# DeepMETv2/DeepMETv2

Measured on AMD Instinct MI355X. Metric: events/sec (4.5k PF cands, k=16), higher is better.
Workload: dtype f32

## Files before the change

### deepmetv2_amd/_lib.py

```python
from __future__ import annotations

import ctypes as C
import os
import threading

_PKG_DIR = os.path.dirname(os.path.abspath(__file__))
LIB_PATH = os.environ.get("DMET_HIP_LIB") or os.path.join(_PKG_DIR, "libdmet_hip.so")

_lock = threading.Lock()
_lib = None

_vp, _i, _i64, _sz, _f, _d = C.c_void_p, C.c_int, C.c_int64, C.c_size_t, C.c_float, C.c_double

SIGNATURES = {
    "dmet_version": (_i, []),
    "dmet_last_error": (C.c_char_p, []),
    "dmet_device_available": (_i, []),
    "dmet_knn_workspace_bytes": (_sz, [_i64, _i, _i, _i]),
    "dmet_knn_f32": (_i, [_vp, _vp, _i, _i64, _i, _i, _vp, _vp, _vp, _sz, _vp]),
    "dmet_knn_local_f32": (_i, [_vp, _vp, _i, _i64, _i, _i, _vp, _vp, _vp, _vp, _sz, _vp]),
    "dmet_knn_periodic_f32": (_i, [_vp, _vp, _i, _i64, _i, _i, _vp, _vp, _vp, _vp, _vp, _sz, _vp]),
    "dmet_knn_xy_workspace_bytes": (_sz, [_i64, _i64, _i, _i, _i]),
    "dmet_knn_xy_f32": (_i, [_vp, _vp, _i64, _vp, _vp, _i64, _i, _i, _i, _vp, _vp, _vp, _vp, _sz, _vp]),
    "dmet_radius_xy_f32": (_i, [_vp, _vp, _i64, _vp, _vp, _i64, _i, _i, _f, _i, _vp, _i, _vp, _vp, _vp]),
    "dmet_edge_features_xy_f32": (_i, [_vp, _vp, _vp, _vp, _i64, _i, _vp, _vp]),
    "dmet_edge_features_xy_bwd_f32": (_i, [_vp, _vp, _vp, _vp, _i64, _i64, _i, _vp, _vp, _vp]),
    "dmet_adamw_f32": (_i, [_vp, _vp, _vp, _vp, _vp, _vp, _i64, _d, _d, _d, _d, _d, _vp]),
    "dmet_adamw_lr_f32": (_i, [_vp, _vp, _vp, _vp, _vp, _vp, _i64, _vp, _d, _d, _d, _d, _vp]),
    "dmet_bn_knn_local_dense_f32": (_i, [_vp, _vp, _vp, _vp, _vp, _vp, _vp, _vp, _i, _i64, _i, _i, _vp, _vp, _vp, _vp, _vp, _i,
                                         _vp, _vp, _vp, _vp, _vp, _sz, _vp]),
    "dmet_knn_local_dense_f32": (_i, [_vp, _vp, _i, _i64, _i, _i, _vp, _vp, _vp, _vp, _vp, _i, _vp, _vp, _vp, _vp, _sz, _vp]),
    "dmet_knn_fallback_stats": (_i, [_vp, _i64, _i, _i, _i, _vp, _vp]),
    "dmet_knn_retry_stats": (_i, [_vp, _i64, _i, _i, _i, _vp, _vp]),
    "dmet_knn_size_hint": (_i, [_i, _i]),
    "dmet_finalize_defer_begin": (_i, []),
    "dmet_finalize_pending": (_i, []),
    "dmet_finalize_flush": (_i, [_vp]),
    "dmet_radius_f32": (_i, [_vp, _vp, _i, _i64, _i, _f, _i, _i, _vp, _vp, _vp]),
    "dmet_radius_counted_f32": (_i, [_vp, _vp, _i, _i64, _i, _f, _i, _i, _vp, _vp, _vp]),
    "dmet_radius_workspace_bytes": (_sz, [_i64]),
    "dmet_radius_windowed_f32": (_i, [_vp, _vp, _i, _i64, _i, _f, _i, _i, _i, _vp, _vp, _vp, _sz, _vp]),
    "dmet_radius_windowed_local_f32": (_i, [_vp, _vp, _i, _i64, _i, _f, _i, _i, _i, _vp, _vp, _vp, _i, _vp, _sz, _vp]),
    "dmet_radius_periodic_f32": (_i, [_vp, _vp, _i, _i64, _i, _f, _i, _i, _i, _vp, _vp, _vp, _vp]),
    "dmet_radius_windowed_periodic_f32": (_i, [_vp, _vp, _i, _i64, _i, _f, _i, _i, _i, _vp, _vp, _vp, _vp, _i, _vp, _sz,
                                               _vp]),
    "dmet_edgeconv_linear_workspace_bytes": (_sz, [_i64, _i]),
    "dmet_edgeconv_linear_max_fwd_f32": (_i, [_vp, _vp, _vp, _i, _i64, _i, _i, _i, _vp, _vp, _vp, _vp, _vp, _sz, _vp]),
    "dmet_edgeconv_fused_lds_f32": (_i, [_vp, _vp, _vp, _i, _i64, _i, _i, _i, _vp, _vp, _vp, _vp, _vp]),
    "dmet_node_linear_split_f32": (_i, [_vp, _i64, _i, _i, _vp, _vp, _vp, _vp, _vp]),
    "dmet_node_linear_split_sliced_f32": (_i, [_vp, _i64, _i, _i, _vp, _vp, _vp, _vp, _vp]),
    "dmet_bn_node_linear_split_f32": (_i, [_vp, _vp, _vp, _vp, _vp, _vp, _vp, _i64, _i, _vp, _vp, _i, _vp, _vp, _vp]),
    "dmet_gather_max_f32": (_i, [_vp, _vp, _vp, _vp, _i, _i64, _i, _i, _vp, _vp, _vp]),
    "dmet_gather_max_counted_f32": (_i, [_vp, _vp, _vp, _vp, _i64, _i, _i, _vp, _vp, _vp]),
    "dmet_gather_max_lds_f32": (_i, [_vp, _vp, _vp, _vp, _i, _i64, _i, _i, _vp, _vp, _vp]),
    "dmet_gather_max_counted_lds_f32": (_i, [_vp, _vp, _vp, _vp, _vp, _i, _i64, _i, _i, _i, _vp, _vp, _vp]),
    "dmet_gather_max_lds_sliced_f32": (_i, [_vp, _vp, _vp, _vp, _vp, _i, _i64, _i, _i, _vp, _vp, _vp]),
    "dmet_gather_max_lds_sliced_cap_f32": (_i, [_vp, _vp, _vp, _vp, _vp, _i, _i64, _i, _i, _vp, _vp, _i64, _vp]),
    "dmet_gather_max_lds16_f32": (_i, [_vp, _vp, _vp, _vp, _vp, _i, _i64, _i, _i, _vp, _vp, _vp]),
    "dmet_edge_mlp2_supported": (_i, [_i, _i, _i, _i]),
    "dmet_edge_mlp2_bf16": (_i, [_vp, _i64, _i, _vp, _i, _vp, _vp, _i, _vp, _vp, _i, _i, _i, _vp, _vp]),
    "dmet_edge_mlp2_bn_workspace_bytes": (_sz, [_i64, _i]),
    "dmet_edge_mlp2_bn_bf16": (_i, [_vp, _i64, _i, _vp, _i, _vp, _vp, _i, _vp, _vp, _i, _i, _i, _vp, _vp, _f, _f, _vp, _vp, _vp,
                                    _i, _vp, _vp, _sz, _vp]),
    "dmet_edge_mlp_f32_supported": (_i, [_i, _i, _i]),
    "dmet_edge_mlp_f32_workspace_bytes": (_sz, [_i64, _i64, _i, _i, _i]),
    "dmet_edge_mlp_fwd_f32": (_i, [_vp, _i64, _i, _vp, _vp, _vp, _i64, _vp, _vp, _i, _vp, _vp, _i, _i, _i, _i, _vp, _vp, _f, _f,
                                   _vp, _vp, _vp, _vp, _vp, _vp, _vp, _vp, _vp, _sz, _vp]),
    "dmet_edge_mlp_bwd_f32": (_i, [_vp, _i64, _i, _vp, _vp, _vp, _i64, _vp, _vp, _vp, _i, _vp, _vp, _i, _i, _i, _i, _vp, _vp,
                                   _vp, _vp, _vp, _vp, _vp, _vp, _vp, _vp, _vp, _vp, _sz, _vp]),
    "dmet_edge_mlp_bf16_supported": (_i, [_i, _i, _i]),
    "dmet_edge_mlp_bf16_workspace_bytes": (_sz, [_i64, _i64, _i, _i, _i]),
    "dmet_edge_mlp_fwd_bf16": (_i, [_vp, _i64, _i, _vp, _vp, _vp, _i64, _vp, _vp, _i, _vp, _vp, _i, _i, _i, _i, _vp, _vp, _f, _f,
                                    _vp, _vp, _vp, _vp, _vp, _vp, _vp, _vp, _vp, _sz, _vp]),
    "dmet_edge_mlp_bwd_bf16": (_i, [_vp, _i64, _i, _vp, _vp, _vp, _i64, _vp, _vp, _vp, _i, _vp, _vp, _i, _i, _i, _i, _vp, _vp,
                                    _vp, _vp, _vp, _vp, _vp, _vp, _vp, _vp, _vp, _vp, _sz, _vp]),
    "dmet_edge_mlp_f16_supported": (_i, [_i, _i, _i]),
    "dmet_edge_mlp_f16_workspace_bytes": (_sz, [_i64, _i64, _i, _i, _i]),
    "dmet_edge_mlp_fwd_f16": (_i, [_vp, _i64, _i, _vp, _vp, _vp, _i64, _vp, _vp, _i, _vp, _vp, _i, _i, _i, _i, _vp, _vp, _f, _f,
                                   _vp, _vp, _vp, _vp, _vp, _vp, _vp, _vp, _vp, _sz, _vp]),
    "dmet_edge_mlp_bwd_f16": (_i, [_vp, _i64, _i, _vp, _vp, _vp, _i64, _vp, _vp, _vp, _i, _vp, _vp, _i, _i, _i, _i, _vp, _vp,
                                   _vp, _vp, _vp, _vp, _vp, _vp, _vp, _vp, _vp, _vp, _sz, _vp]),
    "dmet_table_order_by_count": (_i, [_vp, _vp, _i, _i64, _vp, _vp]),
    "dmet_gather_max_counted_lds_j16_f32": (_i, [_vp, _vp, _vp, _vp, _vp, _vp, _i, _i64, _i, _i, _i, _vp, _vp, _vp]),
    "dmet_gather_max_local_j16_f32": (_i, [_vp, _vp, _vp, _i, _vp, _vp, _vp, _i, _i64, _i, _i, _i, _vp, _vp, _vp]),
    "dmet_gather_max_bwd_j16_f32": (_i, [_vp, _vp, _vp, _i, _i64, _i, _vp, _vp]),
    "dmet_gather_max_mixed_f32": (_i, [_vp, _vp, _vp, _vp, _vp, _i, _i64, _i, _i, _vp, _vp, _vp]),
    "dmet_node_linear_split_bf16": (_i, [_vp, _i64, _i, _i, _vp, _vp, _vp, _vp, _vp]),
    "dmet_gather_max_bf16q": (_i, [_vp, _vp, _vp, _i64, _i, _i, _vp, _vp, _vp]),
    "dmet_gather_max_bwd_f32": (_i, [_vp, _vp, _vp, _vp, _i64, _i, _i, _vp, _vp]),
    "dmet_gather_sum_table_f32": (_i, [_vp, _vp, _vp, _vp, _i64, _i, _i, _i, _vp, _vp, _vp]),
# ... 43 lines not shown
    "dmet_met_loss_f32": (_i, [_vp, _vp, _i, _vp, _vp, _vp]),
    "dmet_met_loss_strided_f32": (_i, [_vp, _vp, _i64, _i, _vp, _vp, _vp]),
    "dmet_met_reduce_bwd_scaled_f32": (_i, [_vp, _vp, _vp, _i64, _vp, _i, _i64, _vp, _vp]),
    "dmet_segment_sum_1d_f32": (_i, [_vp, _vp, _i, _vp, _vp]),
    "dmet_table_degree": (_i, [_vp, _vp, _i64, _i, _vp, _vp]),
    "dmet_table_edges": (_i, [_vp, _vp, _vp, _i64, _i, _i, _vp, _vp, _vp, _vp, _vp]),
    "dmet_batch_to_ptr": (_i, [_vp, _i64, _i, _vp, _vp]),
    "dmet_xty_workspace_bytes": (_sz, [_i64, _i, _i]),
    "dmet_xty_f32": (_i, [_vp, _vp, _i64, _i, _i, _vp, _vp, _sz, _vp]),
    "dmet_onehot_xty_f32": (_i, [_vp, _vp, _i64, _i, _i, _vp, _vp, _sz, _vp]),
    "dmet_gather_max_bwd_lds_f32": (_i, [_vp, _vp, _vp, _vp, _i, _i64, _i, _i, _vp, _vp]),
    "dmet_gather_max_bwd_lds16_f32": (_i, [_vp, _vp, _vp, _vp, _vp, _i, _i64, _i, _i, _vp, _vp]),
    "dmet_gather_max_bwd_lds16_cap_f32": (_i, [_vp, _vp, _vp, _vp, _vp, _i, _i64, _i, _i, _vp, _i64, _vp]),
    "dmet_gather_max_bwd_j16_cap_f32": (_i, [_vp, _vp, _vp, _i, _i64, _i, _vp, _i64, _vp]),
    "dmet_gather_max_bwd_sliced_f32": (_i, [_vp, _vp, _vp, _vp, _vp, _i, _i64, _i, _i, _vp, _i64, _vp]),
    "dmet_gather_max_bwd_j16_sliced_f32": (_i, [_vp, _vp, _vp, _i, _i64, _i, _vp, _i64, _vp]),
    "dmet_edgeconv_linear_bwd_sliced_f32": (_i, [_vp, _vp, _vp, _vp, _i, _vp, _vp, _i64, _i, _vp, _vp, _vp, _vp, _sz, _vp]),
    "dmet_edgeconv_linear_bwd_workspace_bytes": (_sz, [_i64, _i]),
    "dmet_edgeconv_linear_bwd_f32": (_i, [_vp, _vp, _vp, _vp, _vp, _i64, _i, _vp, _vp, _vp, _vp, _sz, _vp]),
    "dmet_edgeconv_linear_bwd_add_f32": (_i, [_vp, _vp, _vp, _vp, _vp, _vp, _i64, _i, _vp, _vp, _vp, _vp, _sz, _vp]),
    "dmet_edgeconv_linear_bwd_add_j16_f32": (_i, [_vp, _vp, _vp, _vp, _vp, _vp, _i64, _i, _vp, _vp, _vp, _vp, _sz, _vp]),
    "dmet_head_fwd_f32": (_i, [_vp, _i64, _vp, _vp, _vp, _vp, _vp, _vp]),
    "dmet_head_bwd_workspace_bytes": (_sz, [_i64]),
    "dmet_head_bwd_f32": (_i, [_vp, _i64] + [_vp] * 10 + [_vp, _sz, _vp]),
    "dmet_bn_workspace_bytes": (_sz, [_i64, _i]),
    "dmet_bn_fwd_f32": (_i, [_vp, _vp, _i64, _i, _vp, _vp, _f, _f, _vp, _vp, _i, _vp, _vp, _vp, _vp, _sz, _vp]),
    "dmet_bn_fwd_tracked_f32": (_i, [_vp, _vp, _i64, _i, _vp, _vp, _f, _f, _vp, _vp, _vp, _i, _vp, _vp, _vp, _vp, _sz, _vp]),
    "dmet_bn_head_fwd_f32": (_i, [_vp, _vp, _vp, _vp, _vp, _vp, _vp, _i64, _vp, _vp, _vp, _vp, _vp, _vp, _vp]),
    "dmet_bn_bwd_stats_f32": (_i, [_vp, _vp, _i64, _i, _vp, _vp, _vp, _vp, _vp, _vp, _vp, _sz, _vp]),
    "dmet_encode_bn_bwd_f32": (_i, [_vp, _i64, _vp, _i64] + [_vp] * 9 + [_vp, _vp] + [_vp] * 5 + [_vp] * 9 + [_vp, _vp, _sz, _vp]),
    "dmet_bn_eval_stats_f32": (_i, [_vp, _vp, _i, _f, _vp, _vp, _vp]),
    "dmet_bn_apply_f32": (_i, [_vp, _vp, _i64, _i, _vp, _vp, _vp, _vp, _vp, _vp]),
    "dmet_bn_stats_f32": (_i, [_vp, _i64, _i, _f, _f, _vp, _vp, _vp, _vp, _vp, _vp, _sz, _vp]),
    "dmet_bn_bwd_f32": (_i, [_vp, _vp, _i64, _i, _vp, _vp, _vp, _vp, _vp, _vp, _vp, _sz, _vp]),
    "dmet_encode_fwd_f32": (_i, [_vp, _i64, _vp, _i64] + [_vp] * 9 + [_vp, _vp]),
    "dmet_encode_bwd_workspace_bytes": (_sz, [_i64]),
    "dmet_encode_bwd_f32": (_i, [_vp, _i64, _vp, _i64] + [_vp] * 9 + [_vp, _vp] + [_vp] * 9 + [_vp, _sz, _vp]),
    "dmet_graclus_workspace_bytes": (_sz, [_i64]),
    "dmet_graclus_f32": (_i, [_vp, _vp, _vp, _vp, _i, _i64, C.c_uint64, _i, _vp, _vp, _vp, _vp, _sz, _vp]),
    "dmet_normalized_cut_workspace_bytes": (_sz, [_i64]),
    "dmet_normalized_cut_f32": (_i, [_vp, _vp, _i64, _i64, _vp, _vp, _vp, _sz, _vp]),
    "dmet_normalized_cut_2d_f32": (_i, [_vp, _vp, _i64, _i64, _vp, _i, _vp, _vp, _sz, _vp]),
    "dmet_pool_pairs_workspace_bytes": (_sz, [_i64, _i]),
    "dmet_pool_pairs_index": (_i, [_vp, _vp, _i, _i64, _vp, _vp, _vp, _sz, _vp]),
    "dmet_pool_pairs_f32": (_i, [_vp, _i64, _i, _vp, _vp, _vp, _i, _i64, _vp, _vp, _vp, _vp, _vp]),
    "dmet_pool_pairs_bwd_f32": (_i, [_vp, _vp, _vp, _vp, _vp, _i64, _i, _i64, _vp, _vp]),
    "dmet_fps_workspace_bytes": (_sz, [_i64, _i, _i]),
    "dmet_fps_f32": (_i, [_vp, _vp, _i, _i64, _i, _vp, _vp, _i64, _vp, _vp, _sz, _vp]),
    "dmet_topk_workspace_bytes": (_sz, [_i64]),
    "dmet_topk_f32": (_i, [_vp, _vp, _i, _i64, _vp, _i64, _vp, _vp, _vp, _sz, _vp]),
    "dmet_select_rows_f32": (_i, [_vp, _vp, _vp, _i64, _i64, _i, _vp, _vp]),
    "dmet_select_rows_bwd_f32": (_i, [_vp, _vp, _vp, _vp, _i64, _i64, _i, _vp, _vp, _vp]),
    "dmet_filter_table": (_i, [_vp, _vp, _vp, _vp, _i64, _i64, _i, _vp, _vp, _vp]),
    "dmet_filter_edges_workspace_bytes": (_sz, [_i64]),
    "dmet_filter_edges_count": (_i, [_vp, _vp, _i64, _vp, _i64, _vp, _vp, _vp, _sz, _vp]),
    "dmet_filter_edges_write": (_i, [_vp, _vp, _i64, _vp, _i64, _vp, _sz, _i64, _vp, _vp, _vp]),
}


class DmetLibraryError(RuntimeError):
    pass


def load() -> C.CDLL:
    global _lib
    if _lib is not None:
# ... 22 lines not shown
```

### deepmetv2_amd/_native.py

```python
from __future__ import annotations

import contextlib
import ctypes
import inspect
import math
import os
from typing import Optional, Tuple

import torch

from . import _lib


def _require_device(*tensors: torch.Tensor) -> torch.device:
    dev = None
    for t in tensors:
        if t is None:
            continue
        if t.device.type != "cuda":
            raise RuntimeError(
                "deepmetv2_amd: operator called with a non-GPU tensor. The HIP extension is the only "
                "implementation (no CPU fallback); move inputs to a ROCm device.")
        if dev is None:
            dev = t.device
# ... 412 lines not shown
    _t = timer.record('node_linear_split', dev)
    with _on(dev):
        _lib.check(L.dmet_bn_node_linear_split_f32(raw.data_ptr(), _ptr(residual), *[v.data_ptr() for v in vec], y.data_ptr(),
                                                   N, 32, W.data_ptr(), _ptr(b), layout, P.data_ptr(), Q.data_ptr(),
                                                   _stream(dev)), "dmet_bn_node_linear_split_f32")
    if _t is not None:
        _t.record(torch.cuda.current_stream(dev))
    return y, P, Q


def _gather_run(dev: torch.device, key: str, note: Optional[str], entry: str, *args) -> None:
    _t = timer.record(key, dev)
    if note is not None:
        _note_gather(note)
    with _on(dev):
        _lib.check(getattr(_lib.load(), entry)(*args, _stream(dev)), entry)
    if _t is not None:
        _t.record(torch.cuda.current_stream(dev))


def _pq_shape(P: torch.Tensor, sliced: bool) -> Tuple[int, int]:
    return (P.shape[1], P.shape[0] * 8) if sliced else (P.shape[0], P.shape[1])


def _check_nbr_local(nbr_local: Optional[torch.Tensor], nbr: torch.Tensor) -> None:
    if nbr_local is not None and (nbr_local.shape != nbr.shape or nbr_local.dtype != torch.int16
                                  or not nbr_local.is_contiguous()):
        raise ValueError("nbr_local must be the contiguous int16 [N, k] table of knn_local()")


def gather_max(P: torch.Tensor, Q: torch.Tensor, nbr: torch.Tensor, ptr: Optional[torch.Tensor],
               want_arg: bool, cnt: Optional[torch.Tensor] = None, lds: bool = False,
               nbr_local: Optional[torch.Tensor] = None, sliced: bool = False, mixed: bool = False,
               max_nodes: Optional[int] = None) -> Tuple[torch.Tensor, Optional[torch.Tensor]]:
    dev = _require_device(P, Q, nbr)
    N, H = _pq_shape(P, sliced)
    k = nbr.shape[1]
    out = torch.empty((N, H), dtype=torch.float32, device=dev)
    arg = torch.empty((N, H), dtype=torch.uint8, device=dev) if want_arg else None
    table = (P.data_ptr(), Q.data_ptr(), nbr.data_ptr())
    local = _ptr(nbr_local)
    events = (ptr.data_ptr(), ptr.numel() - 1) if ptr is not None else (None, 0)
    outs = (out.data_ptr(), arg.data_ptr() if want_arg else None)
    tail = (N, k, H) + outs
    lds_form = ptr is not None and H % 8 == 0 and GATHER_MAX_FORM != "l2-only"
    if mixed and cnt is None and not sliced and ptr is not None and GATHER_MAX_FORM == "auto":
        _check_nbr_local(nbr_local, nbr)
        entry, args = "dmet_gather_max_mixed_f32", table + (local,) + events + tail
        note = ("gather_max_lds_kernel (events <= 5119 nodes: Q slice resident in LDS) + gather_max_mlp_kernel "
                "(larger events: row gathers from L2), chosen per event in one call; row-major P/Q")
    elif sliced and cnt is None:
        if ptr is None or k not in LDS_GATHER_K or GATHER_MAX_FORM == "l2-only":
            raise ValueError("gather_max: slice-major tables are only read by the LDS-resident kernels")
        entry, args = "dmet_gather_max_lds_sliced_cap_f32", table + (local,) + events + tail + (int(max_nodes or 0),)
        note = ("gather_max_lds_kernel (per-event Q slice resident in LDS; slice-major P/Q, "
                + ("uint16 event-local ids)" if nbr_local is not None else "int32 ids)"))
    elif cnt is not None and lds and lds_form:
        entry = "dmet_gather_max_counted_lds_f32"
        args = table + (cnt.data_ptr(),) + events + (N, k, H, 1 if sliced else 0) + outs
        note = ("gather_max_lds_kernel, counted rows (radius table; Q slice resident in LDS"
                + (", slice-major P/Q)" if sliced else ")"))
    elif sliced:
        raise ValueError("gather_max: slice-major tables are only read by the LDS-resident kernels")
    elif cnt is not None:
        entry, args = "dmet_gather_max_counted_f32", table + (cnt.data_ptr(),) + tail
        note = "gather_max_kernel, counted rows (radius table; gathers from L2)"
    elif (lds or GATHER_MAX_FORM == "lds") and lds_form and nbr_local is not None and k in LDS_GATHER_K:
        _check_nbr_local(nbr_local, nbr)
        entry, args = "dmet_gather_max_lds16_f32", table + (local,) + events + tail
        note = "gather_max_lds_kernel (per-event Q slice resident in LDS; row-major P/Q, uint16 ids)"
    elif (lds or GATHER_MAX_FORM == "lds") and lds_form:
        entry, args = "dmet_gather_max_lds_f32", table + events + tail
        note = "gather_max_lds_kernel (per-event Q slice resident in LDS; row-major P/Q, int32 ids)"
    else:
        entry, args = "dmet_gather_max_f32", table + events + tail
        note = "gather_max_mlp_kernel (row gathers from L2; events too large for the LDS image)"
    _gather_run(dev, 'gather_max', note, entry, *args)
    return out, arg


def table_order_by_count(cnt: torch.Tensor, ptr: torch.Tensor) -> torch.Tensor:
    dev = _require_device(cnt, ptr)
    L = _lib.load()
    N = cnt.numel()
    order = torch.empty((N,), dtype=torch.int32, device=dev)
    with _on(dev):
        _lib.check(L.dmet_table_order_by_count(cnt.data_ptr(), ptr.data_ptr(), ptr.numel() - 1, N, order.data_ptr(),
                                               _stream(dev)), "dmet_table_order_by_count")
    return order


def gather_max_counted_j16(P: torch.Tensor, Q: torch.Tensor, nbr: torch.Tensor, cnt: torch.Tensor,
                           order: Optional[torch.Tensor], ptr: torch.Tensor, sliced: bool):
    dev = _require_device(P, Q, nbr, cnt, ptr)
    N, H = _pq_shape(P, sliced)
    k = nbr.shape[1]
    out = torch.empty((N, H), dtype=torch.float32, device=dev)
    argj = torch.empty((N, H), dtype=torch.int16, device=dev)
    _gather_run(dev, 'gather_max', "gather_max_lds_kernel, counted rows (radius table; Q slice resident in LDS, winner ids, "
                "rows ordered by depth" + (", slice-major P/Q)" if sliced else ")"), "dmet_gather_max_counted_lds_j16_f32",
                P.data_ptr(), Q.data_ptr(), nbr.data_ptr(), cnt.data_ptr(), _ptr(order),
                ptr.data_ptr(), ptr.numel() - 1, N, k, H, 1 if sliced else 0, out.data_ptr(), argj.data_ptr())
    return out, argj


def gather_max_local_j16(P: torch.Tensor, Q: torch.Tensor, rows16: torch.Tensor, cnt: torch.Tensor,
                         order: Optional[torch.Tensor], ptr: torch.Tensor, kmax: int, sliced: bool, want_arg: bool = True):
    dev = _require_device(P, Q, rows16, cnt, ptr)
    N, H = _pq_shape(P, sliced)
# ... 1444 lines not shown
                                         ws.numel(), _stream(dev)), "dmet_onehot_xty_f32")
    return C


def _encode_params(params, dev):
    shapes = [(16, 8), (16,), (16, 24), (16,), (32, 32), (32,), (3, 8), (7, 8), (8, 8)]
    if len(params) != 9:
        raise ValueError("encode: expected 9 parameter tensors (Wc, bc, Wk, bk, Wa, ba, Echg, Epdg, Epv)")
    out = []
    for t, shp in zip(params, shapes):
        if tuple(t.shape) != shp:
            raise ValueError(f"encode: parameter of shape {tuple(t.shape)}, expected {shp}")
        if t.device != dev:
            raise ValueError("encode: parameters must be on the device of x")
        out.append(_f32c(t, "param"))
    return out


def _encode_x(x: torch.Tensor, x_cat: torch.Tensor):
    if x.dim() != 2 or x.shape[1] != 8 or x.dtype != torch.float32:
        raise ValueError(f"encode: x_cont must be float32 [N,8], got {tuple(x.shape)} {x.dtype}")
    if x_cat.dim() != 2 or x_cat.shape != (x.shape[0], 3):
        raise ValueError(f"encode: x_cat must be [N,3], got {tuple(x_cat.shape)}")
    if x_cat.dtype == torch.float32:
        if (x.stride(1) == 1 and x_cat.stride(1) == 1 and x_cat.stride(0) == x.stride(0) and x.stride(0) >= 11
                and x_cat.data_ptr() == x.data_ptr() + 32):
            return x, None
        x_cat = x_cat.long()
    if x_cat.dtype != torch.int64:
        raise ValueError(f"encode: x_cat must be int64 (or the float columns 8..10 of x), got {x_cat.dtype}")
    return (x if x.stride(1) == 1 else x.contiguous()), x_cat.contiguous()


def encode_fwd(x_cont: torch.Tensor, x_cat: torch.Tensor, params) -> torch.Tensor:
    dev = _require_device(x_cont, x_cat)
    L = _lib.load()
    x, xc = _encode_x(x_cont, x_cat)
    ps = _encode_params(params, dev)
    N = x.shape[0]
    h = torch.empty((N, 32), dtype=torch.float32, device=dev)
    with _on(dev):
        _lib.check(L.dmet_encode_fwd_f32(x.data_ptr(), x.stride(0), _ptr(xc), N, *[t.data_ptr() for t in ps],
                                         h.data_ptr(), _stream(dev)), "dmet_encode_fwd_f32")
    return h


def encode_bwd(x_cont: torch.Tensor, x_cat: torch.Tensor, params, h: torch.Tensor, g_h: torch.Tensor):
    dev = _require_device(x_cont, x_cat, h, g_h)
    L = _lib.load()
    x, xc = _encode_x(x_cont, x_cat)
    ps = _encode_params(params, dev)
    h = _f32a(h, "h"); g_h = _f32a(g_h, "g_h")
    N = x.shape[0]
    grads = [torch.empty_like(t) for t in ps]
    if N == 0:
        return [g.zero_() for g in grads]
    with _on(dev):
        ws = _ws(L.dmet_encode_bwd_workspace_bytes(N), dev)
        again = _defer_second_use(dev, *params)
        try:
            _lib.check(L.dmet_encode_bwd_f32(x.data_ptr(), x.stride(0), _ptr(xc), N, *[t.data_ptr() for t in ps],
                                             h.data_ptr(), g_h.data_ptr(), *[g.data_ptr() for g in grads], ws.data_ptr(),
                                             ws.numel(), _stream(dev)), "dmet_encode_bwd_f32")
        finally:
            if again:
                _defer_resume()
        _defer_keep(dev, ws, *grads)
    return grads


def encode_bn_bwd(x_cont: torch.Tensor, x_cat: torch.Tensor, params, h: torch.Tensor, g_y: torch.Tensor,
                  gamma: torch.Tensor, mean: torch.Tensor, invstd: torch.Tensor):
    dev = _require_device(x_cont, x_cat, h, g_y)
    L = _lib.load()
    x, xc = _encode_x(x_cont, x_cat)
    ps = _encode_params(params, dev)
    h = _f32c(h, "h"); g_y = _f32c(g_y, "g_y"); gamma = _f32c(gamma.detach(), "gamma")
# ... 34 lines not shown
def bn_fwd(x: torch.Tensor, residual: Optional[torch.Tensor], gamma: torch.Tensor, beta: torch.Tensor, eps: float,
           momentum: float, running_mean: Optional[torch.Tensor], running_var: Optional[torch.Tensor], training: bool,
           num_batches_tracked: Optional[torch.Tensor] = None):
    dev = _require_device(x, gamma, beta)
    L = _lib.load()
    x = _f32a(x, "x")
    N, H = x.shape
    if residual is not None:
        residual = _f32a(residual, "residual")
        if residual.shape != x.shape:
            raise ValueError("bn_fwd: residual must have the shape of x")
    for t in (running_mean, running_var):
        if t is not None and (not t.is_contiguous() or t.dtype != torch.float32 or t.numel() != H):
            raise ValueError("bn_fwd: running statistics must be contiguous float32 [H]")
    gamma = _f32a(gamma, "gamma"); beta = _f32a(beta, "beta")
    y = torch.empty_like(x)
    stats = torch.empty((2, H), dtype=torch.float32, device=dev)
    with _on(dev):
        ws = _ws(L.dmet_bn_workspace_bytes(N, H), dev)
        nbt = None
        if num_batches_tracked is not None and training:
            if num_batches_tracked.dtype != torch.int64 or num_batches_tracked.numel() != 1 or num_batches_tracked.device != dev:
                raise ValueError("bn_fwd: num_batches_tracked must be an int64 scalar on x's device")
            nbt = num_batches_tracked.data_ptr()
        _lib.check(L.dmet_bn_fwd_tracked_f32(x.data_ptr(), _ptr(residual), N, H, gamma.data_ptr(), beta.data_ptr(),
                                             float(eps), float(momentum), _ptr(running_mean), _ptr(running_var), nbt,
                                             1 if training else 0, y.data_ptr(), stats[0].data_ptr(),
                                             stats[1].data_ptr(), ws.data_ptr(), ws.numel(), _stream(dev)),
                   "dmet_bn_fwd_tracked_f32")
    return y, stats[0], stats[1]


def bn_stats(x: torch.Tensor, eps: float, momentum: float, running_mean: Optional[torch.Tensor],
             running_var: Optional[torch.Tensor], num_batches_tracked: Optional[torch.Tensor] = None):
    dev = _require_device(x)
    L = _lib.load()
    x = _f32a(x, "x")
    N, H = x.shape
    stats = torch.empty((2, H), dtype=torch.float32, device=dev)
    with _on(dev):
        ws = _ws(L.dmet_bn_workspace_bytes(N, H), dev)
        _lib.check(L.dmet_bn_stats_f32(x.data_ptr(), N, H, float(eps), float(momentum), _ptr(running_mean),
                                       _ptr(running_var), _ptr(num_batches_tracked),
                                       stats[0].data_ptr(), stats[1].data_ptr(), ws.data_ptr(), ws.numel(), _stream(dev)),
                   "dmet_bn_stats_f32")
    return stats[0], stats[1]


def bn_apply(x: torch.Tensor, residual: Optional[torch.Tensor], gamma: torch.Tensor, beta: torch.Tensor,
             mean: torch.Tensor, invstd: torch.Tensor) -> torch.Tensor:
    dev = _require_device(x, gamma, beta, mean, invstd)
    L = _lib.load()
    x, residual, vec, aligned = _bn_affine_operands("bn_apply", x, residual, gamma, beta, mean, invstd)
    if not aligned:
        x, vec = _aligned16(x), [_aligned16(v) for v in vec]
        residual = _aligned16(residual) if residual is not None else None
    N, H = x.shape
    y = torch.empty_like(x)
    with _on(dev):
        _lib.check(L.dmet_bn_apply_f32(x.data_ptr(), _ptr(residual), N, H, *[v.data_ptr() for v in vec], y.data_ptr(),
                                       _stream(dev)), "dmet_bn_apply_f32")
    return y


def bn_eval_stats(running_mean: torch.Tensor, running_var: torch.Tensor, eps: float):
    dev = _require_device(running_mean, running_var)
    L = _lib.load()
    H = running_mean.numel()
    stats = torch.empty((2, H), dtype=torch.float32, device=dev)
    with _on(dev):
        _lib.check(L.dmet_bn_eval_stats_f32(running_mean.data_ptr(), running_var.data_ptr(), H, float(eps),
                                            stats[0].data_ptr(), stats[1].data_ptr(), _stream(dev)), "dmet_bn_eval_stats_f32")
    return stats[0], stats[1]


def bn_knn_local_dense(raw: torch.Tensor, residual: Optional[torch.Tensor], gamma: torch.Tensor, beta: torch.Tensor,
                       mean: torch.Tensor, invstd: torch.Tensor, ptr: torch.Tensor, k: int, dense=None):
    dev = _require_device(raw, ptr)
# ... 501 lines not shown
```

### deepmetv2_amd/conv.py

```python
from __future__ import annotations

import os
from typing import Callable, Optional, Tuple, Union

import torch

from . import _native
from .cluster import fp16_autocast, knn_table, knn_xy_table
from .graph import BipartiteTable, EdgeList, GraphFuture, NeighborTable, batch_info, edge_list_from_edge_index, lookup_graph
from .scatter import _SegmentMaxRows, _SegmentSumRows
from torch.autograd.function import once_differentiable

_FUSED_WIDTHS = (32, 64)


def _reset(nn_module) -> None:
    if hasattr(nn_module, "reset_parameters"):
        nn_module.reset_parameters()
    elif hasattr(nn_module, "children"):
        for child in nn_module.children():
            _reset(child)


def _as_fusable_linear(nn_module) -> Optional[torch.nn.Linear]:
# ... 55 lines not shown
            if pq is not None and pq[2] is sliced and pq[0].shape[-2 if sliced else 0] == x.shape[0]:
                P, Q = pq[0], pq[1]
            else:
                P, Q = _native.node_linear_split(x, weight, bias, sliced=sliced)
            table.join()
            auto = lds and _native.GATHER_MAX_FORM == "auto"
            ctx.j16 = auto and need_grad and table.nonempty and os.environ.get("DMET_RADIUS_J16", "1") != "0"
            rows16 = table.rows16 is not None and os.environ.get("DMET_RADIUS_IDS", "rows16") == "rows16"
            if ctx.j16 and rows16:
                out, arg = _native.gather_max_local_j16(P, Q, table.rows16, table.cnt, table.order_by_count(), table.ptr,
                                                        table.k, sliced)
            elif ctx.j16:
                out, arg = _native.gather_max_counted_j16(P, Q, table.nbr, table.cnt, table.order_by_count(), table.ptr,
                                                          sliced)
            elif auto and not need_grad and rows16:
                out, arg = _native.gather_max_local_j16(P, Q, table.rows16, table.cnt, table.order_by_count(), table.ptr,
                                                        table.k, sliced, want_arg=False)
            else:
                out, arg = _native.gather_max(P, Q, table.nbr, table.ptr, want_arg=need_grad, cnt=table.cnt, lds=lds,
                                              sliced=sliced)
        elif EDGECONV_FORM == "fused" and _lds_eligible(x, weight, table):
            out, arg = _native.edgeconv_fused_lds(x, weight, bias, table.nbr, table.ptr, want_arg=need_grad)
        else:
            lds = _lds_eligible(x, weight, table)
            mixed = (not lds and _lds_eligible(x, weight, table, any_size=True) and table.max_nodes is not None
                     and os.environ.get("DMET_GATHER_MIXED", "0") == "1")
            sliced = _pq_sliced(lds)
            pq = table.pq
            table.pq = None
            if pq is not None and pq[2] is sliced and pq[0].shape[-2 if sliced else 0] == x.shape[0]:
                P, Q = pq[0], pq[1]
            else:
                P, Q = _native.node_linear_split(x, weight, bias, sliced=sliced)
            out, arg = _native.gather_max(P, Q, table.nbr, table.ptr, want_arg=need_grad, lds=lds,
                                          nbr_local=table.nbr_local, sliced=sliced, mixed=mixed, max_nodes=table.max_nodes)
        if need_grad:
            ctx.save_for_backward(x, weight, arg)
            ctx.table = table
            ctx.has_bias = bias is not None
        if passthrough:
            return out, x.view_as(x)
        return out

    @staticmethod
    def backward(ctx, g_out, g_pass=None):
        _native.no_double_backward("_EdgeConvLinearMax")
        x, weight, arg = ctx.saved_tensors
        table: NeighborTable = ctx.table
        H = x.shape[1]
        g_out = g_out.contiguous()
        fused_node = H == 32 and tuple(weight.shape) == (32, 64) and g_out.dtype == torch.float32
        gqs = fused_node and os.environ.get("DMET_GQ_SLICED", "1") != "0"
        if ctx.j16:
            gQ = _native.gather_max_bwd_j16(g_out, arg, table.ptr, max_nodes=table.max_nodes, sliced=gqs)
        elif H == 32 and g_out.dtype == torch.float32 and table.ptr is not None and GATHER_BWD_FORM != "reverse":
            gQ = _native.gather_max_bwd_lds(g_out, arg, table.nbr, table.ptr, nbr_local=table.nbr_local,
                                            max_nodes=table.max_nodes, sliced=gqs)
        else:
            gqs = False
            rev_ptr, rev_pos = table.reverse()
            gQ = _native.gather_max_bwd(g_out, arg, rev_ptr, rev_pos, table.k)
        if fused_node:
            gx, gW, gb = _native.edgeconv_linear_bwd(x, weight.detach(), g_out,
                                                     None if table.dense else arg, gQ,
                                                     want_bias=ctx.has_bias, g_add=g_pass, gq_sliced=gqs)
            return (gx if ctx.needs_input_grad[0] else None, gW if ctx.needs_input_grad[1] else None,
                    gb if (ctx.has_bias and ctx.needs_input_grad[2]) else None, None, None, None)
        none = 0xFFFF if ctx.j16 else 255
# ... 463 lines not shown
        return f"{self.__class__.__name__}(nn={self.nn})"


class DynamicEdgeConv(EdgeConv):

    def __init__(self, nn: Callable, k: int, aggr: str = "max", num_workers: int = 1, **kwargs):
        super().__init__(nn=nn, aggr=aggr, **kwargs)
        if not isinstance(k, int) or k < 1:
            raise ValueError(f"k must be a positive int, got {k!r}")
        self.k = k
        self.num_workers = num_workers

    def forward(self, x: Union[torch.Tensor, Tuple[torch.Tensor, torch.Tensor]],
                batch: Union[None, torch.Tensor, Tuple[torch.Tensor, torch.Tensor]] = None) -> torch.Tensor:
        if isinstance(x, (tuple, list)):
            if x[1] is not None and x[1] is not x[0]:
                x_src, x_dst = self._check_features(x[0], "x_src"), self._check_features(x[1], "x_dst")
                b_src, b_dst = batch if isinstance(batch, (tuple, list)) else (batch, batch)
                return self._forward_pair(x_src, x_dst, knn_xy_table(x_src, x_dst, self.k, b_src, b_dst))
            x = x[0]
        if isinstance(batch, (tuple, list)):
            batch = batch[0]
        if x.dim() != 2:
            raise ValueError("Static graphs not supported in DynamicEdgeConv")
        if x.dtype == torch.bfloat16 or (x.dtype == torch.float16 and self._takes_fp16()):
            x = x.float()
        if x.dtype != torch.float32:
            raise TypeError(f"x must be float32, got {x.dtype}")
        table = self._take_prebuilt(x)
        if table is None:
            table = knn_table(x, self.k, batch, loop=True, dense=self._dense_request(x))
        return self._forward_table(x, table)

    def forward_with_residual_input(self, x: torch.Tensor, batch: Optional[torch.Tensor] = None):
        if x.dim() != 2 or x.dtype != torch.float32:
            return self.forward(x, batch), x
        table = self._take_prebuilt(x)
        if table is None:
            table = knn_table(x, self.k, batch, loop=True, dense=self._dense_request(x))
        return self._forward_table(x, table, passthrough=True)

    def prebuild_hook(self, batch: Optional[torch.Tensor] = None, graph=None):
        if BN_KNN_FUSE == "0" or self.k > 20 or os.environ.get("DMET_KNN_PATH") == "exact":
            return None

        def build(raw, residual, gamma, beta, mean, invstd):
            if not raw.is_cuda or raw.dim() != 2 or raw.shape[1] != 32 or raw.dtype != torch.float32:
                return None
            info = batch_info(batch, raw.shape[0], raw.device)
            req = self._dense_request(raw)
            dense = (req[0], req[1], req[2](info.max_nodes)) if req is not None else None
            _native.knn_size_hint(info.min_nodes, info.max_nodes)
            out = _native.bn_knn_local_dense(raw, residual, gamma, beta, mean, invstd, info.ptr, self.k, dense)
            if out is None:
                return None
            y, nbr, dist, loc, pq = out
            table = NeighborTable(nbr, info.ptr, dense=False, dist=dist, max_nodes=info.max_nodes, nbr_local=loc)
            table.pq = pq
            self._prebuilt = (y, table)
            return y
        return build

    def _take_prebuilt(self, x: torch.Tensor):
        pre, self._prebuilt = getattr(self, "_prebuilt", None), None
        if pre is not None and pre[0].data_ptr() == x.data_ptr() and pre[0].shape == x.shape:
            return pre[1]
        return None

    def _dense_request(self, x: torch.Tensor):
        if KNN_RIDER == "0" or self.aggr != "max" or EDGECONV_FORM != "split" or x.shape[1] != 32 or not x.is_cuda:
            return None
        lin = _as_fusable_linear(self.nn)
        if lin is None or lin.in_features != 64 or lin.out_features != 32 or self.k not in _native.LDS_GATHER_K:
# ... 13 lines not shown
```

### deepmetv2_amd/csrc/common.h

```cpp
#pragma once
#include <hip/hip_runtime.h>
#include <stdint.h>
#include <stdio.h>
#include <stdlib.h>
#include <string.h>

#include <type_traits>

#include "../../include/dmet.h"

namespace dmet {

constexpr int kWave = 64;
constexpr int kNumXcd = 8;
constexpr float kKnnSentinel = 1e10f;

void set_error(const char *fmt, ...);
int hip_fail(hipError_t e, const char *what);

#define DMET_REQUIRE(cond, ...)                 \
    do {                                        \
        if (!(cond)) {                          \
            ::dmet::set_error(__VA_ARGS__);     \
            return -22;                         \
// ... 23 lines not shown
        const int mid = (lo + hi) >> 1;
        if (ptr[mid] <= i) lo = mid; else hi = mid;
    }
    return lo;
}

__device__ __forceinline__ int xcd_swizzle(int bid, int nblk)
{
    const int q = nblk / kNumXcd, rm = nblk % kNumXcd;
    const int xcd = bid % kNumXcd, idx = bid / kNumXcd;
    const int base = (xcd < rm) ? xcd * (q + 1) : rm * (q + 1) + (xcd - rm) * q;
    return base + idx;
}

constexpr int kEcbPartialFloats = 2 * 1024 + 32;
constexpr int kEncPartialFloats = 3 * 1024 + 64;
constexpr int kHeadPartialFloats = 1024 + 64;
enum { kDeferEdgeConv = 0, kDeferEncoder = 1, kDeferHead = 2 };
struct DeferDesc {
    int kind;
    const float *partial;
    int64_t nparts;
    float *out[9];
};
bool defer_push(const DeferDesc &d);

__device__ __forceinline__ float wave_sum(float v)
{
#pragma unroll
    for (int off = 32; off > 0; off >>= 1) v += __shfl_xor(v, off, 64);
    return v;
}

template <int... Vs, typename F>
bool with_int(int v, F &&f)
{
    return ((v == Vs && (f(std::integral_constant<int, Vs>{}), true)) || ...);
}
template <typename F>
void with_flags(F &&f) { f(); }
template <typename F, typename... Rest>
void with_flags(F &&f, bool b, Rest... rest)
{
    if (b) with_flags([&](auto... c) { f(std::true_type{}, c...); }, rest...);
    else with_flags([&](auto... c) { f(std::false_type{}, c...); }, rest...);
}

}
```

### deepmetv2_amd/csrc/edgeconv.hip

```cpp
#include <stdlib.h>

#include <hip/hip_bf16.h>

#include <type_traits>

#include "common.h"
#include "nls_body.h"

namespace dmet {
namespace {

typedef float f32x16 __attribute__((ext_vector_type(16)));

template <int HIN, int HOUT, bool SLICED = false>
__global__ __launch_bounds__(256) void node_linear_split_kernel(const float *__restrict__ x, int64_t N,
                                                                 const float *__restrict__ W,
                                                                 const float *__restrict__ bias,
                                                                 float *__restrict__ P, float *__restrict__ Q)
{
    __shared__ __attribute__((aligned(16))) float tpose[SLICED ? 4 : 1][SLICED ? kNlsLdsFloats : 1];
    const int wv = __builtin_amdgcn_readfirstlane(threadIdx.x >> 6);
    const int64_t wave = (int64_t)blockIdx.x * (blockDim.x >> 6) + wv;
    const int64_t nwaves = (int64_t)gridDim.x * (blockDim.x >> 6);
    node_linear_split_wave<HIN, HOUT, SLICED>(x, N, W, bias, P, Q, tpose[SLICED ? wv : 0], wave, nwaves, threadIdx.x & 63);
// ... 243 lines not shown
    }
    int4 mine[K4 / 2];
#pragma unroll
    for (int q = 0; q < K4 / 2; ++q) mine[q] = row4[half * (K4 / 2) + q];
#pragma unroll
    for (int q = 0; q < K4 / 2; ++q) {
        int4 other;
        other.x = dpp_swap_pair(mine[q].x); other.y = dpp_swap_pair(mine[q].y);
        other.z = dpp_swap_pair(mine[q].z); other.w = dpp_swap_pair(mine[q].w);
        ids[q] = half ? other : mine[q];
        ids[K4 / 2 + q] = half ? mine[q] : other;
    }
}

template <int K4>
__device__ __forceinline__ void load_ids16_pair(unsigned (&w)[K4], const uint16_t *__restrict__ row, int half)
{
    const unsigned *src = reinterpret_cast<const unsigned *>(row) + half * K4;
    if (K4 % 4 == 0) {
#pragma unroll
        for (int q = 0; q < K4 / 4; ++q) {
            const uint4 v = reinterpret_cast<const uint4 *>(src)[q];
            w[4 * q] = v.x; w[4 * q + 1] = v.y; w[4 * q + 2] = v.z; w[4 * q + 3] = v.w;
        }
    } else if (K4 == 2) {
        const uint2 v = *reinterpret_cast<const uint2 *>(src);
        w[0] = v.x; w[1] = v.y;
    } else {
#pragma unroll
        for (int q = 0; q < K4; ++q) w[q] = src[q];
    }
}

template <bool WITH_ARG, int K4, int GML_MODE, bool IDS16, bool SLICED, int ROWS = kLdsGatherRows, int THREADS = kLdsGatherThreads>
__device__ __forceinline__ void gather_max_lds_segment(
    float4 *__restrict__ qs, const float *__restrict__ P, const float *__restrict__ Q, const int32_t *__restrict__ nbr,
    const uint16_t *__restrict__ nbr16, const int64_t *__restrict__ ptr, int k, int H,
    float *__restrict__ out, uint8_t *__restrict__ arg, int64_t N, int skip_big, const int b, const int sl, const int i0,
    const int i1)
{
    static_assert(K4 >= 1 && K4 <= 8, "k = 4 K4 <= 32");
    constexpr int RPI = THREADS / 2;
    const int lo = (int)ptr[b], hi = (int)ptr[b + 1];
    const int n = hi - lo;
    if (n <= 0 || i0 >= i1) return;
    const int h4 = H / 4;
    const float4 *Q4 = reinterpret_cast<const float4 *>(Q);
    const float4 *P4 = reinterpret_cast<const float4 *>(P);
    const int half = threadIdx.x & 1;
    const int r0 = i0 + (threadIdx.x >> 1);
    const int col4 = sl * 2 + half;
    const float ninf = -__builtin_inff();
    auto pq_at = [&](const int64_t i) -> int64_t { return SLICED ? ((int64_t)sl * N + i) * 2 + half : i * h4 + col4; };

    if (n + 1 > ROWS) {
        if (skip_big) return;
        for (int r = r0; r < i1; r += RPI) {
            const int64_t node = lo + r;
            float4 best = make_float4(ninf, ninf, ninf, ninf);
            int a0 = 255, a1 = 255, a2 = 255, a3 = 255;
            bool any = false;
            for (int s = 0; s < k; ++s) {
                const int j = nbr[node * k + s];
                if (j < 0) continue;
                any = true;
                const float4 v = Q4[pq_at(j)];
                if (v.x > best.x) { best.x = v.x; a0 = s; }
                if (v.y > best.y) { best.y = v.y; a1 = s; }
                if (v.z > best.z) { best.z = v.z; a2 = s; }
                if (v.w > best.w) { best.w = v.w; a3 = s; }
            }
            float4 o = make_float4(0.f, 0.f, 0.f, 0.f);
            if (any) {
                const float4 p = P4[pq_at(node)];
                o = make_float4(p.x + best.x, p.y + best.y, p.z + best.z, p.w + best.w);
            }
            reinterpret_cast<float4 *>(out)[node * h4 + col4] = o;
            if (WITH_ARG)
                reinterpret_cast<uchar4 *>(arg)[node * h4 + col4] =
                    make_uchar4((unsigned char)a0, (unsigned char)a1, (unsigned char)a2, (unsigned char)a3);
        }
        return;
    }

    if (GML_MODE != 1) {
        const int lane = threadIdx.x & 63, wave = threadIdx.x >> 6;
        const int nchunk = (n + 31) / 32;
        for (int c = wave; c < nchunk; c += THREADS / 64) {
            int row = 32 * c + (lane >> 1);
            row = min(row, n - 1);
            const float4 *src = SLICED ? Q4 + ((int64_t)sl * N + lo + row) * 2 + (lane & 1)
                                       : Q4 + (int64_t)(lo + row) * h4 + sl * 2 + (lane & 1);
            __builtin_amdgcn_global_load_lds((const __attribute__((address_space(1))) void *)src,
                                             (__attribute__((address_space(3))) void *)(qs + 64 * c), 16, 0, 0);
        }
    }
    int4 ids[K4];
    unsigned idw[K4];
    float4 pv = make_float4(0.f, 0.f, 0.f, 0.f);
    if (r0 < i1) {
        if constexpr (IDS16) {
            load_ids16_pair<K4>(idw, nbr16 + (int64_t)(lo + r0) * k, half);
        } else {
            const int4 *row4 = reinterpret_cast<const int4 *>(nbr + (int64_t)(lo + r0) * k);
            load_ids_pair<K4>(ids, row4, half);
        }
        pv = P4[pq_at(lo + r0)];
    }
    __builtin_amdgcn_s_waitcnt(0);
    __syncthreads();
    if (threadIdx.x < 2) qs[n * 2 + threadIdx.x] = make_float4(ninf, ninf, ninf, ninf);
    __syncthreads();

    for (int r = r0; r < i1; r += RPI) {
        const int64_t node = lo + r;
        unsigned off[4 * K4];
        if constexpr (IDS16) {
#pragma unroll
            for (int q = 0; q < K4; ++q) {
                const unsigned mine = idw[q], other = (unsigned)dpp_swap_pair((int)mine);
                const unsigned a = half ? other : mine, c = half ? mine : other;
                off[2 * q] = min(a & 0xFFFFu, (unsigned)n) * 2 + half;
                off[2 * q + 1] = min(a >> 16, (unsigned)n) * 2 + half;
                off[2 * K4 + 2 * q] = min(c & 0xFFFFu, (unsigned)n) * 2 + half;
                off[2 * K4 + 2 * q + 1] = min(c >> 16, (unsigned)n) * 2 + half;
            }
        } else {
#pragma unroll
            for (int q = 0; q < K4; ++q) {
                off[4 * q + 0] = min((unsigned)(ids[q].x - lo), (unsigned)n) * 2 + half;
                off[4 * q + 1] = min((unsigned)(ids[q].y - lo), (unsigned)n) * 2 + half;
                off[4 * q + 2] = min((unsigned)(ids[q].z - lo), (unsigned)n) * 2 + half;
                off[4 * q + 3] = min((unsigned)(ids[q].w - lo), (unsigned)n) * 2 + half;
            }
        }
        const float4 p = pv;
        if (r + RPI < i1) {
            if constexpr (IDS16) {
                load_ids16_pair<K4>(idw, nbr16 + (node + RPI) * k, half);
            } else {
                const int4 *row4 = reinterpret_cast<const int4 *>(nbr + (node + RPI) * k);
                load_ids_pair<K4>(ids, row4, half);
            }
            pv = P4[pq_at(node + RPI)];
        }
// ... 42 lines not shown
        for (int q0 = 0; q0 < (GML_MODE == 2 ? 0 : K4); q0 += 2) {
            float4 v[8];
            constexpr int kLastSlot = 4 * K4 - 1;
#pragma unroll
            for (int u = 0; u < 8; ++u) v[u] = qs[off[min(4 * q0 + u, kLastSlot)]];
#pragma unroll
            for (int u = 0; u < 8; ++u) {
                if (4 * q0 + u > kLastSlot) continue;
                if (WITH_ARG) {
                    switch (4 * q0 + u) {
#define DMET_CASE(S_) case S_: DMET_MAX_ARG(bx, a0, v[u].x, S_); DMET_MAX_ARG(by, a1, v[u].y, S_); \
                               DMET_MAX_ARG(bz, a2, v[u].z, S_); DMET_MAX_ARG(bw, a3, v[u].w, S_); break;
                        DMET_CASE(0) DMET_CASE(1) DMET_CASE(2) DMET_CASE(3) DMET_CASE(4) DMET_CASE(5) DMET_CASE(6)
                        DMET_CASE(7) DMET_CASE(8) DMET_CASE(9) DMET_CASE(10) DMET_CASE(11) DMET_CASE(12)
                        DMET_CASE(13) DMET_CASE(14) DMET_CASE(15) DMET_CASE(16) DMET_CASE(17) DMET_CASE(18)
                        DMET_CASE(19) DMET_CASE(20) DMET_CASE(21) DMET_CASE(22) DMET_CASE(23) DMET_CASE(24)
                        DMET_CASE(25) DMET_CASE(26) DMET_CASE(27) DMET_CASE(28) DMET_CASE(29) DMET_CASE(30)
                        DMET_CASE(31)
#undef DMET_CASE
                    }
                } else if ((u & 1) == 0) {
                    asm("v_max3_f32 %0, %0, %1, %2" : "+v"(bx) : "v"(v[u].x), "v"(v[u + 1].x));
                    asm("v_max3_f32 %0, %0, %1, %2" : "+v"(by) : "v"(v[u].y), "v"(v[u + 1].y));
                    asm("v_max3_f32 %0, %0, %1, %2" : "+v"(bz) : "v"(v[u].z), "v"(v[u + 1].z));
                    asm("v_max3_f32 %0, %0, %1, %2" : "+v"(bw) : "v"(v[u].w), "v"(v[u + 1].w));
                }
            }
        }
        }
        const bool any = WITH_ARG ? (a0 != 255) : (bx > ninf);
        float4 o = make_float4(0.f, 0.f, 0.f, 0.f);
        if (any) o = make_float4(p.x + bx, p.y + by, p.z + bz, p.w + bw);
        reinterpret_cast<float4 *>(out)[node * h4 + col4] = o;
        if (WITH_ARG) {
            const uchar4 a = make_uchar4((unsigned char)a0, (unsigned char)a1, (unsigned char)a2, (unsigned char)a3);
            reinterpret_cast<uchar4 *>(arg)[node * h4 + col4] = a;
        }
    }
}

inline int num_cus()
{
    static int cached = 0;
    if (cached == 0) {
        int dev = 0, cus = 0;
        if (hipGetDevice(&dev) == hipSuccess &&
            hipDeviceGetAttribute(&cus, hipDeviceAttributeMultiprocessorCount, dev) == hipSuccess && cus > 0)
            cached = cus;
        else
            cached = 256;
    }
    return cached;
}

template <bool WITH_ARG, int K4, int GML_MODE = 0, bool IDS16 = false, bool SLICED = false, int ROWS = kLdsGatherRows,
          int THREADS = kLdsGatherThreads>
__global__ __launch_bounds__(THREADS) void gather_max_lds_kernel(
    const float *__restrict__ P, const float *__restrict__ Q, const int32_t *__restrict__ nbr,
    const uint16_t *__restrict__ nbr16, const int64_t *__restrict__ ptr, int B, int k, int H,
    float *__restrict__ out, uint8_t *__restrict__ arg, int64_t N, int skip_big, int balanced)
{
    __shared__ __attribute__((aligned(16))) float4 qs[ROWS * 2];
    const int nsl = H / kSliceC;
    if (!balanced) {
        const int grp = blockIdx.x / (kNumXcd * nsl), rem = blockIdx.x % (kNumXcd * nsl);
        const int b = grp * kNumXcd + (rem % kNumXcd);
        const int sl = rem / kNumXcd;
        if (b >= B) return;
        gather_max_lds_segment<WITH_ARG, K4, GML_MODE, IDS16, SLICED, ROWS, THREADS>(qs, P, Q, nbr, nbr16, ptr, k, H, out, arg, N,
                                                                                      skip_big, b, sl, 0, (int)(ptr[b + 1] - ptr[b]));
        return;
    }
    const int64_t L = (int64_t)nsl * N;
    const int c = xcd_swizzle((int)blockIdx.x, (int)gridDim.x);
    int64_t pos = L * c / gridDim.x;
    const int64_t end = L * (c + 1) / gridDim.x;
    while (pos < end) {
        int b0 = 0, b1 = B;
        while (b1 - b0 > 1) {
            const int mid = (b0 + b1) >> 1;
            if ((int64_t)nsl * ptr[mid] <= pos) b0 = mid; else b1 = mid;
        }
        const int64_t lo = ptr[b0];
        const int n = (int)(ptr[b0 + 1] - lo);
        const int64_t rel = pos - (int64_t)nsl * lo;
        const int sl = (int)(rel / n), i0 = (int)(rel - (int64_t)sl * n);
        const int i1 = (int)((end - pos) < (int64_t)(n - i0) ? i0 + (end - pos) : n);
        gather_max_lds_segment<WITH_ARG, K4, GML_MODE, IDS16, SLICED, ROWS, THREADS>(qs, P, Q, nbr, nbr16, ptr, k, H, out, arg, N,
                                                                                      skip_big, b0, sl, i0, i1);
        pos += i1 - i0;
        __syncthreads();
    }
}

template <bool WITH_ARG, bool SLICED, bool ARGJ = false, bool LOC16 = false>
__global__ __launch_bounds__(kLdsGatherThreads) void gather_max_lds_counted_kernel(
    const float *__restrict__ P, const float *__restrict__ Q, const int32_t *__restrict__ nbr,
    const int32_t *__restrict__ cnt, const int64_t *__restrict__ ptr, int B, int kmax, int H,
    float *__restrict__ out, uint8_t *__restrict__ arg, int64_t N, const int32_t *__restrict__ order = nullptr,
    const uint16_t *__restrict__ nbr16 = nullptr, int stride16 = 0)
{
    __shared__ __attribute__((aligned(16))) float4 qs[kLdsGatherRows * 2];
    constexpr int RPI = kLdsGatherThreads / 2;
    const int nsl = H / kSliceC;
    const int grp = blockIdx.x / (kNumXcd * nsl), rem = blockIdx.x % (kNumXcd * nsl);
// ... 553 lines not shown

namespace {

constexpr int kLdsGatherRowsHalf = kLdsGatherRows / 2;
constexpr int kLdsGatherThreadsHalf = kLdsGatherThreads / 2;

enum GatherFamily {
    kGatherL2,
    kGatherLds,
    kGatherCountedLds
};

struct GatherMax {
    const char *entry;
    GatherFamily family;
    const float *P, *Q;
    int64_t N;
    int k, H;
    float *out;
    dmet_stream_t stream;
    const int32_t *nbr = nullptr;
    const uint16_t *nbr16 = nullptr;
    bool rows16 = false;
    int stride16 = 0;
    const int32_t *cnt = nullptr;
    const int32_t *order = nullptr;
    const int64_t *ptr = nullptr;
    int B = 0;
    void *arg = nullptr;
    bool arg16 = false;
    bool pq_sliced = false;
    int skip_big = 0;
    int64_t max_nodes = 0;
};

int gather_max_launch(const GatherMax &r)
{
    const int64_t N = r.N;
    const int k = r.k, H = r.H, B = r.B;
    const bool k_mlp = k == 8 || k == 16 || k == 32, k_lds = k_mlp || k == 20;
    const GatherFamily fam = (r.skip_big && !(H == 32 && k_mlp && B != 0)) ? kGatherL2 : r.family;
    DMET_REQUIRE(N >= 0 && N < (int64_t)2147483647, "%s: N out of range", r.entry);
    DMET_REQUIRE(k >= 1 && k <= 255, "%s: k=%d not in [1,255] (arg is uint8, 255 = none)", r.entry, k);
    DMET_REQUIRE(!r.rows16 || (r.stride16 >= k && r.stride16 % 8 == 0), "%s: kmax=%d stride16=%d", r.entry, k, r.stride16);
    DMET_REQUIRE(r.max_nodes >= 0, "%s: max_nodes=%lld", r.entry, (long long)r.max_nodes);
    DMET_REQUIRE(fam == kGatherL2 || (H >= kSliceC && H % kSliceC == 0 && H <= DMET_MAX_H), "%s: H=%d must be a multiple of %d",
                 r.entry, H, kSliceC);
    if (N == 0 || (fam != kGatherL2 && B == 0)) return 0;
    const void *table = r.rows16 ? static_cast<const void *>(r.nbr16) : r.nbr;
    DMET_REQUIRE(r.P && r.Q && table && r.out && (fam == kGatherL2 || r.ptr) && (fam != kGatherCountedLds || r.cnt) &&
                     (r.arg || !r.arg16 || r.rows16),
                 "%s: null pointer", r.entry);
    DMET_REQUIRE(aligned16(r.P) && aligned16(r.Q) && aligned16(r.out) && (fam != kGatherLds || aligned16(r.nbr)) &&
                     (fam == kGatherL2 || aligned16(r.nbr16)) && (!r.arg16 || (reinterpret_cast<uintptr_t>(r.arg) & 7u) == 0),
                 "%s: pointers must be 16-B (uint16 winners: 8-B) aligned", r.entry);
    hipStream_t st = as_stream(r.stream);
    uint8_t *arg = static_cast<uint8_t *>(r.arg);
    const int nsl = H / kSliceC;
    const int64_t per_event = (int64_t)((B + kNumXcd - 1) / kNumXcd) * kNumXcd * nsl;

    auto launch_mlp = [&](bool only_big) {
        with_int<8, 16, 32>(k, [&](auto kk) {
            constexpr int K4 = decltype(kk)::value / 4;
            with_flags([&](auto with_arg, auto big) {
                hipLaunchKernelGGL((gather_max_mlp_kernel<32, with_arg(), K4, big()>), dim3((unsigned)((N + 31) / 32)), dim3(256),
                                   0, st, r.P, r.Q, r.nbr, N, r.out, arg, r.ptr, B, kLdsGatherRows);
            }, arg != nullptr, only_big);
        });
    };

    if (fam == kGatherCountedLds) {
        with_flags([&](auto with_arg, auto sliced, auto ids, auto loc16) {
            if constexpr (ids() ? (with_arg() || loc16()) : !loc16())
                hipLaunchKernelGGL((gather_max_lds_counted_kernel<with_arg(), sliced(), ids(), loc16()>),
                                   dim3((unsigned)per_event), dim3(kLdsGatherThreads), 0, st, r.P, r.Q, r.nbr, r.cnt, r.ptr, B, k, H,
                                   r.out, arg, N, r.order, r.nbr16, r.stride16);
        }, arg != nullptr, r.pq_sliced, r.arg16, r.rows16);
        DMET_LAUNCH_CHECK(!r.arg16 ? "gather_max_lds_counted_kernel" : !r.rows16 ? "gather_max_lds_counted_kernel (winner ids)"
                          : arg     ? "gather_max_lds_counted_kernel (uint16 rows)"
                                    : "gather_max_lds_counted_kernel (uint16 rows, no winners)");
        return 0;
    }
    if (fam == kGatherLds && k_lds) {
        const bool half = r.pq_sliced && r.nbr16 && r.max_nodes > 0 && r.max_nodes + 1 <= kLdsGatherRowsHalf &&
                          !env_is("DMET_GATHER_HALF_IMAGE", "0");
        const int cus = num_cus();
        const int64_t units = (int64_t)B * nsl;
        int balanced = units * 16 <= (int64_t)cus * 9 || (units > cus && units % cus != 0 && units % cus <= cus / 8);
        if (const char *e = getenv("DMET_GATHER_BALANCED")) balanced = atoi(e) != 0;
        if (half) balanced = 0;
        int64_t blocks = per_event;
        if (balanced) {
            blocks = cus;
            const int64_t most = ((int64_t)nsl * N + 63) / 64;
            if (blocks > most) blocks = most;
        }
        bool timed = false;
#ifdef DMET_KNN_EXPERIMENT
        const char *e = (!half && arg && r.nbr16 && k == 16) ? getenv("DMET_GML_MODE") : nullptr;
        timed = with_int<1, 2>(e ? atoi(e) : 0, [&](auto mode) {
            hipLaunchKernelGGL((gather_max_lds_kernel<true, 4, decltype(mode)::value, true>), dim3((unsigned)blocks),
                               dim3(kLdsGatherThreads), 0, st, r.P, r.Q, r.nbr, r.nbr16, r.ptr, B, k, H, r.out, arg, N, r.skip_big,
                               balanced);
        });
#endif
        if (!timed)
            with_int<8, 16, 20, 32>(k, [&](auto kk) {
                constexpr int K4 = decltype(kk)::value / 4;
                with_flags([&](auto with_arg, auto ids16, auto sliced, auto small) {
                    constexpr int ROWS = small() ? kLdsGatherRowsHalf : kLdsGatherRows;
                    constexpr int THREADS = small() ? kLdsGatherThreadsHalf : kLdsGatherThreads;
                    if constexpr (!small() || (ids16() && sliced()))
                        hipLaunchKernelGGL((gather_max_lds_kernel<with_arg(), K4, 0, ids16(), sliced(), ROWS, THREADS>),
                                           dim3((unsigned)blocks), dim3(THREADS), 0, st, r.P, r.Q, r.nbr, r.nbr16, r.ptr, B, k, H, r.out,
                                           arg, N, r.skip_big, balanced);
                }, arg != nullptr, r.nbr16 != nullptr, r.pq_sliced, half);
            });
        DMET_LAUNCH_CHECK(half ? "gather_max_lds_kernel (80 KB image)" : "gather_max_lds_kernel");
        if (!r.skip_big) return 0;
        launch_mlp(true);
        DMET_LAUNCH_CHECK("gather_max_mlp_kernel (large events)");
        return 0;
    }
    DMET_REQUIRE(!r.pq_sliced, "%s: k=%d (slice-major tables need k in {8,16,20,32})", r.entry, k);
    bool built = true;
    if (H == 32 && !r.cnt && k_mlp && aligned16(r.nbr))
        launch_mlp(false);
    else
        built = with_int<16, 32, 64, 128>(H, [&](auto hh) {
            constexpr int HH = decltype(hh)::value, NPB = 256 / (HH / 4);
            with_flags([&](auto with_arg) {
                hipLaunchKernelGGL((gather_max_kernel<HH, with_arg()>), dim3((unsigned)((N + NPB - 1) / NPB)), dim3(256), 0, st, r.P,
                                   r.Q, r.nbr, r.cnt, N, k, r.out, arg);
            }, arg != nullptr);
        });
    DMET_REQUIRE(built, "%s: unsupported H=%d (16/32/64/128)", r.entry, H);
    DMET_LAUNCH_CHECK("gather_max_kernel");
    return 0;
}

}

extern "C" int dmet_gather_max_f32(const float *P, const float *Q, const int32_t *nbr, const int64_t *ptr, int B,
                                   int64_t N, int k, int H, float *out, uint8_t *arg, dmet_stream_t stream)
{
    (void)ptr; (void)B;
    GatherMax r{"dmet_gather_max_f32", kGatherL2, P, Q, N, k, H, out, stream};
    r.nbr = nbr; r.arg = arg;
    return gather_max_launch(r);
// ... 18 lines not shown
extern "C" int dmet_gather_max_lds16_f32(const float *P, const float *Q, const int32_t *nbr, const uint16_t *nbr_local,
                                         const int64_t *ptr, int B, int64_t N, int k, int H, float *out,
                                         uint8_t *arg, dmet_stream_t stream)
{
    GatherMax r{"dmet_gather_max_lds16_f32", kGatherLds, P, Q, N, k, H, out, stream};
    r.nbr = nbr; r.nbr16 = nbr_local; r.ptr = ptr; r.B = B; r.arg = arg;
    return gather_max_launch(r);
}

extern "C" int dmet_gather_max_mixed_f32(const float *P, const float *Q, const int32_t *nbr, const uint16_t *nbr_local,
                                         const int64_t *ptr, int B, int64_t N, int k, int H, float *out,
                                         uint8_t *arg, dmet_stream_t stream)
{
    GatherMax r{"dmet_gather_max_mixed_f32", kGatherLds, P, Q, N, k, H, out, stream};
    r.nbr = nbr; r.nbr16 = nbr_local; r.ptr = ptr; r.B = B; r.arg = arg; r.skip_big = 1;
    return gather_max_launch(r);
}

extern "C" int dmet_gather_max_lds_sliced_f32(const float *P, const float *Q, const int32_t *nbr,
                                              const uint16_t *nbr_local, const int64_t *ptr, int B, int64_t N, int k,
                                              int H, float *out, uint8_t *arg, dmet_stream_t stream)
{
    GatherMax r{"dmet_gather_max_lds_sliced_f32", kGatherLds, P, Q, N, k, H, out, stream};
    r.nbr = nbr; r.nbr16 = nbr_local; r.ptr = ptr; r.B = B; r.arg = arg; r.pq_sliced = true;
    return gather_max_launch(r);
}

extern "C" int dmet_gather_max_lds_sliced_cap_f32(const float *P, const float *Q, const int32_t *nbr,
                                                  const uint16_t *nbr_local, const int64_t *ptr, int B, int64_t N, int k,
                                                  int H, float *out, uint8_t *arg, int64_t max_nodes, dmet_stream_t stream)
{
    GatherMax r{"dmet_gather_max_lds_sliced_cap_f32", kGatherLds, P, Q, N, k, H, out, stream};
    r.nbr = nbr; r.nbr16 = nbr_local; r.ptr = ptr; r.B = B; r.arg = arg; r.pq_sliced = true; r.max_nodes = max_nodes;
    return gather_max_launch(r);
}

extern "C" int dmet_gather_max_counted_lds_f32(const float *P, const float *Q, const int32_t *nbr, const int32_t *cnt,
                                               const int64_t *ptr, int B, int64_t N, int k, int H, int pq_sliced,
                                               float *out, uint8_t *arg, dmet_stream_t stream)
{
    GatherMax r{"dmet_gather_max_counted_lds_f32", kGatherCountedLds, P, Q, N, k, H, out, stream};
    r.nbr = nbr; r.cnt = cnt; r.ptr = ptr; r.B = B; r.arg = arg; r.pq_sliced = pq_sliced != 0;
    return gather_max_launch(r);
}

extern "C" int dmet_gather_max_counted_lds_j16_f32(const float *P, const float *Q, const int32_t *nbr, const int32_t *cnt,
                                                   const int32_t *order, const int64_t *ptr, int B, int64_t N, int k,
                                                   int H, int pq_sliced, float *out, uint16_t *argj,
                                                   dmet_stream_t stream)
{
    GatherMax r{"dmet_gather_max_counted_lds_j16_f32", kGatherCountedLds, P, Q, N, k, H, out, stream};
    r.nbr = nbr; r.cnt = cnt; r.order = order; r.ptr = ptr; r.B = B; r.arg = argj; r.arg16 = true; r.pq_sliced = pq_sliced != 0;
    return gather_max_launch(r);
}

extern "C" int dmet_gather_max_local_j16_f32(const float *P, const float *Q, const uint16_t *nbr16, int stride16,
                                             const int32_t *cnt, const int32_t *order, const int64_t *ptr, int B,
                                             int64_t N, int kmax, int H, int pq_sliced, float *out, uint16_t *argj,
                                             dmet_stream_t stream)
{
    GatherMax r{"dmet_gather_max_local_j16_f32", kGatherCountedLds, P, Q, N, kmax, H, out, stream};
    r.nbr16 = nbr16; r.rows16 = true; r.stride16 = stride16; r.cnt = cnt; r.order = order; r.ptr = ptr; r.B = B;
    r.arg = argj; r.arg16 = true; r.pq_sliced = pq_sliced != 0;
    return gather_max_launch(r);
}

// ... 261 lines not shown
```

### deepmetv2_amd/csrc/encoder.hip

```cpp
#include <stdlib.h>

#include "bn_affine.h"
#include "common.h"

namespace dmet {
namespace {

typedef float f32x16 __attribute__((ext_vector_type(16)));

#define ENC_PARAMS                                                                                                  \
    const float *__restrict__ Wc, const float *__restrict__ bc, const float *__restrict__ Wk,                      \
        const float *__restrict__ bk, const float *__restrict__ Wa, const float *__restrict__ ba,                  \
        const float *__restrict__ Echg, const float *__restrict__ Epdg, const float *__restrict__ Epv
#define ENC_ARGS Wc, bc, Wk, bk, Wa, ba, Echg, Epdg, Epv

__device__ __forceinline__ float elu(float z) { return z > 0.0f ? z : (__expf(z) - 1.0f); }

__device__ __forceinline__ void cat_indices(const int64_t *__restrict__ xcat, const float *__restrict__ row, int64_t i,
                                            int &ichg, int &ipdg, int &ipv)
{
    long long c = xcat ? xcat[i * 3 + 0] : (long long)row[8];
    const long long chg = xcat ? xcat[i * 3 + 1] : (long long)row[9];
    const long long pv = xcat ? xcat[i * 3 + 2] : (long long)row[10];
    c = c < 0 ? -c : c;
// ... 27 lines not shown
        z2[o] = b;
    }
#pragma unroll
    for (int o = 0; o < 16; ++o) { joint[o] = elu(z2[o]); joint[16 + o] = elu(z1[o]); }
#pragma unroll
    for (int o = 0; o < 32; ++o) {
        float a = ba[o];
#pragma unroll
        for (int f = 0; f < 32; ++f) a = __builtin_fmaf(Wa[o * 32 + f], joint[f], a);
        z3[o] = a;
    }
}

__global__ __launch_bounds__(256, 2) void encode_fwd_kernel(const float *__restrict__ x, int64_t x_stride,
                                                          const int64_t *__restrict__ xcat, int64_t N,
                                                          ENC_PARAMS, float *__restrict__ h)
{
    const int64_t i = (int64_t)blockIdx.x * blockDim.x + threadIdx.x;
    if (i >= N) return;
    const float *row = x + i * x_stride;
    float xc[8];
#pragma unroll
    for (int f = 0; f < 8; ++f) xc[f] = row[f];
    int ichg, ipdg, ipv;
    cat_indices(xcat, row, i, ichg, ipdg, ipv);
    float cat24[24], z1[16], z2[16], joint[32], z3[32];
    encode_node(ENC_ARGS, xc, ichg, ipdg, ipv, cat24, z1, z2, joint, z3);
    float4 *o = reinterpret_cast<float4 *>(h + i * 32);
#pragma unroll
    for (int c = 0; c < 8; ++c)
        o[c] = make_float4(elu(z3[4 * c]), elu(z3[4 * c + 1]), elu(z3[4 * c + 2]), elu(z3[4 * c + 3]));
}

__global__ __launch_bounds__(256) void encode_fwd_mfma_kernel(const float *__restrict__ x, int64_t x_stride,
                                                               const int64_t *__restrict__ xcat, int64_t N, ENC_PARAMS,
                                                               float *__restrict__ h)
{
    const int lane = threadIdx.x & 63, r = lane & 31, hh = lane >> 5;
    const int64_t wave = (int64_t)blockIdx.x * (blockDim.x >> 6) + __builtin_amdgcn_readfirstlane((int)(threadIdx.x >> 6));
    const int64_t nwaves = (int64_t)gridDim.x * (blockDim.x >> 6);
    const int64_t ntiles = (N + 31) / 32;
    float w12[16], w3[16], b12[16], b3[16];
#pragma unroll
    for (int s = 0; s < 16; ++s) {
        const int f = (s & 3) + 8 * (s >> 2) + 4 * hh;
        const float *src = r < 16 ? Wk + r * 24 + min(f, 23) : Wc + (r - 16) * 8 + max(f - 24, 0);
        const bool keep = r < 16 ? f < 24 : f >= 24;
        const float a = *src;
        w12[s] = keep ? a : 0.0f;
        w3[s] = Wa[r * 32 + f];
        const float *bsrc = f < 16 ? bk + f : bc + (f - 16);
        b12[s] = *bsrc;
        b3[s] = ba[f];
    }
    struct Raw { float c[4]; long long k0, k1, k2; };
    auto load_raw = [&](const int64_t tile, Raw &q) __attribute__((always_inline)) {
        const int64_t node = tile * 32 + r;
        const int64_t i = node < N ? node : N - 1;
        const float *row = x + i * x_stride;
#pragma unroll
        for (int u = 0; u < 4; ++u) q.c[u] = row[4 * hh + u];
        if (xcat) { q.k0 = xcat[i * 3 + 0]; q.k1 = xcat[i * 3 + 1]; q.k2 = xcat[i * 3 + 2]; }
        else { q.k0 = (long long)row[8]; q.k1 = (long long)row[9]; q.k2 = (long long)row[10]; }
    };
    auto load_tables = [&](const Raw &q, float (&in)[16]) __attribute__((always_inline)) {
        long long c = q.k0 < 0 ? -q.k0 : q.k0;
        const long long table[7] = {1, 2, 11, 13, 22, 130, 211};
#pragma unroll
        for (int t = 0; t < 7; ++t) c = (c == table[t]) ? (long long)t : c;
        const int ipdg = (int)min(max(c, 0ll), 6ll), ichg = (int)min(max(q.k1 + 1, 0ll), 2ll), ipv = (int)min(max(q.k2, 0ll), 7ll);
        const float4 e0 = *reinterpret_cast<const float4 *>(Echg + ichg * 8 + 4 * hh);
        const float4 e1 = *reinterpret_cast<const float4 *>(Epdg + ipdg * 8 + 4 * hh);
        const float4 e2 = *reinterpret_cast<const float4 *>(Epv + ipv * 8 + 4 * hh);
        in[0] = e0.x; in[1] = e0.y; in[2] = e0.z; in[3] = e0.w; in[4] = e1.x; in[5] = e1.y; in[6] = e1.z; in[7] = e1.w;
        in[8] = e2.x; in[9] = e2.y; in[10] = e2.z; in[11] = e2.w;
#pragma unroll
        for (int u = 0; u < 4; ++u) in[12 + u] = q.c[u];
    };
    Raw raw;
    float in[16], nxt[16];
    if (wave < ntiles) { load_raw(wave, raw); load_tables(raw, in); }
    if (wave + nwaves < ntiles) load_raw(wave + nwaves, raw);
    for (int64_t tile = wave; tile < ntiles; tile += nwaves) {
        const int64_t node = tile * 32 + r;
        if (tile + nwaves < ntiles) load_tables(raw, nxt);
        if (tile + 2 * nwaves < ntiles) load_raw(tile + 2 * nwaves, raw);
        f32x16 acc;
#pragma unroll
        for (int e = 0; e < 16; ++e) acc[e] = b12[e];
#pragma unroll
        for (int s = 0; s < 16; ++s) acc = __builtin_amdgcn_mfma_f32_32x32x2f32(w12[s], in[s], acc, 0, 0, 0);
        float joint[16];
#pragma unroll
        for (int e = 0; e < 16; ++e) joint[e] = elu(acc[e]);
#pragma unroll
        for (int e = 0; e < 16; ++e) acc[e] = b3[e];
#pragma unroll
        for (int s = 0; s < 16; ++s) acc = __builtin_amdgcn_mfma_f32_32x32x2f32(w3[s], joint[s], acc, 0, 0, 0);
        if (node < N) {
            float4 *o = reinterpret_cast<float4 *>(h + node * 32 + 4 * hh);
#pragma unroll
            for (int g = 0; g < 4; ++g)
                o[2 * g] = make_float4(elu(acc[4 * g]), elu(acc[4 * g + 1]), elu(acc[4 * g + 2]), elu(acc[4 * g + 3]));
        }
#pragma unroll
        for (int u = 0; u < 16; ++u) in[u] = nxt[u];
    }
}

constexpr int kEncTiles = 3;
constexpr int kEncBwdWaves = 4;
constexpr int kEncPartial = kEncTiles * 1024 + 64;

__device__ __forceinline__ void enc_wave_sync()
{
    __builtin_amdgcn_fence(__ATOMIC_RELEASE, "wavefront");
    __builtin_amdgcn_wave_barrier();
    __builtin_amdgcn_fence(__ATOMIC_ACQUIRE, "wavefront");
}

__device__ __forceinline__ void tile_mma(f32x16 &acc, const float *__restrict__ A, const float *__restrict__ Bm, int lane)
{
    const int c = lane & 31, hh = lane >> 5;
#pragma unroll 8
    for (int s = 0; s < 32; ++s) {
        const int node = 2 * s + hh;
        acc = __builtin_amdgcn_mfma_f32_32x32x2f32(A[node * 33 + c], Bm[node * 33 + c], acc, 0, 0, 0);
    }
}

__device__ __forceinline__ void tile_mma_onehot(f32x16 &acc, const int *__restrict__ packed, const float *__restrict__ Bm,
                                                int lane)
{
    const int c = lane & 31, hh = lane >> 5;
    int sh, mask, tgt;
    if (c < 3) { sh = 0; mask = 3; tgt = c; }
    else if (c < 10) { sh = 2; mask = 7; tgt = c - 3; }
    else if (c < 18) { sh = 5; mask = 7; tgt = c - 10; }
    else { sh = 0; mask = 0; tgt = 1; }
#pragma unroll 8
// ... 389 lines not shown
    s = 0.0f;
#pragma unroll
    for (int q = 0; q < 32; ++q) s += red[q][e];
    const int t = idx / 1024, r = (idx % 1024) / 32, c = idx % 32;
    if (t == 0) g.Wa[r * 32 + c] = s;
    else if (t == 1) {
        if (r < 16 && c < 24) g.Wk[r * 24 + c] = s;
        else if (r >= 16 && c >= 24) g.Wc[(r - 16) * 8 + (c - 24)] = s;
    } else if (t == 2) {
        if (r < 3 && c < 8) g.Echg[r * 8 + c] = s;
        else if (r >= 3 && r < 10 && c >= 8 && c < 16) g.Epdg[(r - 3) * 8 + (c - 8)] = s;
        else if (r >= 10 && r < 18 && c >= 16 && c < 24) g.Epv[(r - 10) * 8 + (c - 16)] = s;
    } else if (r == 0) g.ba[c] = s;
    else if (c < 16) g.bk[c] = s;
    else g.bc[c - 16] = s;
}

inline int64_t enc_nodes_per_wave(int64_t N, int64_t *nwaves)
{
    const int64_t target_waves = 2048;
    int64_t npw = (N + target_waves - 1) / target_waves;
#ifdef DMET_ENC_NPW_UP
    npw = (npw + 63) / 64 * 64;
#else
    npw = npw / 64 * 64;
#endif
    if (npw < 64) npw = 64;
    int64_t nw = (N + npw - 1) / npw;
    nw = (nw + kEncBwdWaves - 1) / kEncBwdWaves * kEncBwdWaves;
    *nwaves = nw;
    return npw;
}

thread_local EncBnBwd g_enc_bnb{nullptr, nullptr, nullptr, nullptr, nullptr};
thread_local bool g_enc_bnb_done = false;

}
}

using namespace dmet;

extern "C" int dmet_encode_fwd_f32(const float *x, int64_t x_stride, const int64_t *xcat, int64_t N, const float *Wc, const float *bc,
                                   const float *Wk, const float *bk, const float *Wa, const float *ba,
                                   const float *Echg, const float *Epdg, const float *Epv, float *h,
                                   dmet_stream_t stream)
{
    DMET_REQUIRE(N >= 0 && x_stride >= 8, "dmet_encode_fwd_f32: bad sizes");
    if (N == 0) return 0;
    DMET_REQUIRE(x && Wc && bc && Wk && bk && Wa && ba && Echg && Epdg && Epv && h, "dmet_encode_fwd_f32: null pointer");
    DMET_REQUIRE(xcat || x_stride >= 11, "dmet_encode_fwd_f32: x_cat == NULL needs rows of at least 11 columns (x_stride=%lld)", (long long)x_stride);
    DMET_REQUIRE(aligned16(h), "dmet_encode_fwd_f32: h must be 16-B aligned");
    const int64_t blocks = (N + 255) / 256;
    DMET_REQUIRE(blocks < (1ll << 31), "dmet_encode_fwd_f32: too many nodes");
    const int form = env_is("DMET_ENCODER_FWD", "valu") ? 0 : 1;
    if (form == 1 && aligned16(Echg) && aligned16(Epdg) && aligned16(Epv)) {
        const int64_t tiles = (N + 31) / 32;
        int64_t grid = (tiles + 3) / 4;
        int gmax = 512;
        if (const char *e = getenv("DMET_ENC_GRID")) { gmax = atoi(e); if (gmax < 1) gmax = 512; }
        if (grid > gmax) grid = gmax;
        hipLaunchKernelGGL(encode_fwd_mfma_kernel, dim3((unsigned)grid), dim3(256), 0, as_stream(stream), x, x_stride, xcat, N,
                           ENC_ARGS, h);
        DMET_LAUNCH_CHECK("encode_fwd_mfma_kernel");
        return 0;
    }
    hipLaunchKernelGGL(encode_fwd_kernel, dim3((unsigned)blocks), dim3(256), 0, as_stream(stream), x, x_stride, xcat, N, ENC_ARGS, h);
    DMET_LAUNCH_CHECK("encode_fwd_kernel");
    return 0;
}

extern "C" size_t dmet_encode_bwd_workspace_bytes(int64_t N)
{
    if (N <= 0) return 0;
    int64_t nw;
    (void)enc_nodes_per_wave(N, &nw);
    return sizeof(float) * (size_t)nw * kEncPartial + 512;
}

extern "C" int dmet_encode_bwd_f32(const float *x, int64_t x_stride, const int64_t *xcat, int64_t N, const float *Wc, const float *bc,
                                   const float *Wk, const float *bk, const float *Wa, const float *ba,
                                   const float *Echg, const float *Epdg, const float *Epv, const float *h,
                                   const float *g_h, float *gWc, float *gbc, float *gWk, float *gbk, float *gWa,
                                   float *gba, float *gEchg, float *gEpdg, float *gEpv, void *ws, size_t ws_bytes,
                                   dmet_stream_t stream)
{
    DMET_REQUIRE(N > 0 && x_stride >= 8, "dmet_encode_bwd_f32: bad sizes");
    DMET_REQUIRE((xcat || x_stride >= 11) && x && Wc && bc && Wk && bk && Wa && ba && Echg && Epdg && Epv && h && g_h && gWc && gbc && gWk && gbk &&
                     gWa && gba && gEchg && gEpdg && gEpv && ws,
                 "dmet_encode_bwd_f32: null pointer");
    DMET_REQUIRE(ws_bytes >= dmet_encode_bwd_workspace_bytes(N), "dmet_encode_bwd_f32: workspace too small");
    DMET_REQUIRE(aligned16(h) && aligned16(g_h), "dmet_encode_bwd_f32: h / g_h must be 16-B aligned");
    int64_t nw;
    const int64_t npw = enc_nodes_per_wave(N, &nw);
    float *partial = reinterpret_cast<float *>((reinterpret_cast<uintptr_t>(ws) + 255u) & ~(uintptr_t)255u);
    hipStream_t st = as_stream(stream);
    const int form = env_is("DMET_ENCODER_BWD", "valu") ? 0 : 1;
    int64_t nparts = nw / kEncBwdWaves;
    if (form == 1 && aligned16(Echg) && aligned16(Epdg) && aligned16(Epv) && aligned16(g_h) && aligned16(h)) {
        const int64_t tiles = (N + 31) / 32;
        int64_t grid = (tiles + kEncBwdWaves - 1) / kEncBwdWaves;
// ... 54 lines not shown
```

### deepmetv2_amd/csrc/norm.hip

```cpp
#include "bn_affine.h"
#include "common.h"

namespace dmet {
namespace {

constexpr int kBnBlocks = 512;
constexpr int kBnThreads = 256;

template <int MODE>
__global__ __launch_bounds__(kBnThreads) void bn_reduce_kernel(const float *__restrict__ x, const float *__restrict__ g,
                                                               int64_t N, int H, const float *__restrict__ stat_a,
                                                               const float *__restrict__ stat_b, int64_t rows_per_block,
                                                               float *__restrict__ partial)
{
    __shared__ float4 red0[kBnThreads], red1[kBnThreads];
    const int h4 = H / 4;
    const int rpb = kBnThreads / h4;
    const int tid = threadIdx.x;
    const int c4 = tid % h4, rr = tid / h4;
    const int64_t lo = (int64_t)blockIdx.x * rows_per_block, hi = min(N, lo + rows_per_block);
    float4 a = make_float4(0.f, 0.f, 0.f, 0.f), b = a;
    float4 sa = a, sb = make_float4(1.f, 1.f, 1.f, 1.f);
    if (rr < rpb) {
        if (MODE == 0) sa = reinterpret_cast<const float4 *>(x)[c4];
// ... 44 lines not shown
    __syncthreads();
    s0 = 0.0; s1 = 0.0;
    if (grp == 0)
        for (int q = 0; q < 16; ++q) { s0 += g0[q][c]; s1 += g1[q][c]; }
}

__global__ __launch_bounds__(1024) void bn_fwd_finalize_kernel(const float *__restrict__ partial, int nblocks,
                                                             const float *__restrict__ x, int64_t N, int H, float eps,
                                                             float momentum, float *__restrict__ running_mean,
                                                             float *__restrict__ running_var,
                                                             float *__restrict__ save_mean,
                                                             float *__restrict__ save_invstd,
                                                             int64_t *__restrict__ num_batches_tracked)
{
    double s0, s1;
    bn_combine(partial, nblocks, H, s0, s1);
    const int c = threadIdx.x;
    if (c == 0 && num_batches_tracked) *num_batches_tracked += 1;
    if (c >= H) return;
    const double shift = (double)x[c];
    const double m = s0 / (double)N;
    double var = s1 / (double)N - m * m;
    if (var < 0.0) var = 0.0;
    const double mean = shift + m;
    save_mean[c] = (float)mean;
    save_invstd[c] = (float)(1.0 / sqrt(var + (double)eps));
    if (running_mean) {
        const double unbiased = N > 1 ? var * (double)N / (double)(N - 1) : var;
        running_mean[c] = (float)((1.0 - (double)momentum) * (double)running_mean[c] + (double)momentum * mean);
        running_var[c] = (float)((1.0 - (double)momentum) * (double)running_var[c] + (double)momentum * unbiased);
    }
}

__global__ __launch_bounds__(64) void bn_eval_stats_kernel(const float *__restrict__ running_mean,
                                                           const float *__restrict__ running_var, int H, float eps,
                                                           float *__restrict__ save_mean,
                                                           float *__restrict__ save_invstd)
{
    const int c = threadIdx.x;
    if (c >= H) return;
    save_mean[c] = running_mean[c];
    save_invstd[c] = (float)(1.0 / sqrt((double)running_var[c] + (double)eps));
}

__global__ __launch_bounds__(256) void bn_apply_kernel(const float *__restrict__ x, const float *__restrict__ res,
                                                       int64_t N, int H, const float *__restrict__ gamma,
                                                       const float *__restrict__ beta, const float *__restrict__ mean,
                                                       const float *__restrict__ invstd, float *__restrict__ y)
{
    const BnAffine a{x, res, gamma, beta, mean, invstd};
    const int h4 = H / 4;
    const int64_t total = N * h4;
    for (int64_t t = (int64_t)blockIdx.x * blockDim.x + threadIdx.x; t < total; t += (int64_t)gridDim.x * blockDim.x) {
        const float4 v = reinterpret_cast<const float4 *>(x)[t];
        const BnAffine4 c = bn_affine_load4(a, (int)(t % h4));
        float4 o = bn_affine4(v, c.mu, c.scale, c.beta);
        if (res) o = bn_add4(o, reinterpret_cast<const float4 *>(res)[t]);
        reinterpret_cast<float4 *>(y)[t] = o;
    }
}

__global__ __launch_bounds__(1024) void bn_bwd_finalize_kernel(const float *__restrict__ partial, int nblocks, int64_t N,
                                                             int H, float *__restrict__ g_gamma,
                                                             float *__restrict__ g_beta, float *__restrict__ mean_g,
                                                             float *__restrict__ mean_gx)
{
// ... 72 lines not shown
                           (const float *)nullptr, (const float *)nullptr, rpb, partial);
        DMET_LAUNCH_CHECK("bn_reduce_kernel<0>");
        hipLaunchKernelGGL(bn_fwd_finalize_kernel, dim3(1), dim3(1024), 0, st, partial, nb, x, N, H, eps, momentum,
                           running_mean, running_var, save_mean, save_invstd, num_batches_tracked);
        DMET_LAUNCH_CHECK("bn_fwd_finalize_kernel");
    } else {
        hipLaunchKernelGGL(bn_eval_stats_kernel, dim3(1), dim3(64), 0, st, (const float *)running_mean,
                           (const float *)running_var, H, eps, save_mean, save_invstd);
        DMET_LAUNCH_CHECK("bn_eval_stats_kernel");
    }
    return dmet_bn_apply_f32(x, residual, N, H, gamma, beta, save_mean, save_invstd, y, stream);
}

extern "C" int dmet_bn_stats_f32(const float *x, int64_t N, int H, float eps, float momentum, float *running_mean,
                                 float *running_var, int64_t *num_batches_tracked, float *save_mean, float *save_invstd,
                                 void *ws, size_t ws_bytes, dmet_stream_t stream)
{
    DMET_REQUIRE(bn_shape_ok(H), "dmet_bn_stats_f32: H=%d must be a multiple of 4 in [4,64]", H);
    DMET_REQUIRE(N > 0, "dmet_bn_stats_f32: N=%lld", (long long)N);
    DMET_REQUIRE(x && save_mean && save_invstd && ws, "dmet_bn_stats_f32: null pointer");
    DMET_REQUIRE(aligned16(x) && aligned16(save_mean) && aligned16(save_invstd), "dmet_bn_stats_f32: pointers must be 16-byte aligned");
    DMET_REQUIRE(ws_bytes >= dmet_bn_workspace_bytes(N, H), "dmet_bn_stats_f32: workspace too small");
    DMET_REQUIRE((running_mean == nullptr) == (running_var == nullptr), "dmet_bn_stats_f32: running_mean/var go together");
    hipStream_t st = as_stream(stream);
    float *partial = reinterpret_cast<float *>((reinterpret_cast<uintptr_t>(ws) + 255u) & ~(uintptr_t)255u);
    int64_t rpb;
    const int nb = bn_blocks(N, &rpb);
    hipLaunchKernelGGL((bn_reduce_kernel<0>), dim3(nb), dim3(kBnThreads), 0, st, x, (const float *)nullptr, N, H,
                       (const float *)nullptr, (const float *)nullptr, rpb, partial);
    DMET_LAUNCH_CHECK("bn_reduce_kernel<0>");
    hipLaunchKernelGGL(bn_fwd_finalize_kernel, dim3(1), dim3(1024), 0, st, partial, nb, x, N, H, eps, momentum, running_mean,
                       running_var, save_mean, save_invstd, num_batches_tracked);
    DMET_LAUNCH_CHECK("bn_fwd_finalize_kernel");
    return 0;
}

extern "C" int dmet_bn_fwd_f32(const float *x, const float *residual, int64_t N, int H, const float *gamma,
                               const float *beta, float eps, float momentum, float *running_mean, float *running_var,
                               int training, float *y, float *save_mean, float *save_invstd, void *ws, size_t ws_bytes,
                               dmet_stream_t stream)
{
    return dmet_bn_fwd_tracked_f32(x, residual, N, H, gamma, beta, eps, momentum, running_mean, running_var, nullptr,
                                   training, y, save_mean, save_invstd, ws, ws_bytes, stream);
}

extern "C" int dmet_bn_bwd_f32(const float *x, const float *g_y, int64_t N, int H, const float *gamma,
                               const float *save_mean, const float *save_invstd, float *g_x, float *g_gamma,
                               float *g_beta, void *ws, size_t ws_bytes, dmet_stream_t stream)
{
    DMET_REQUIRE(bn_shape_ok(H), "dmet_bn_bwd_f32: H=%d must be a multiple of 4 in [4,64]", H);
    DMET_REQUIRE(N > 0, "dmet_bn_bwd_f32: N=%lld", (long long)N);
    DMET_REQUIRE(x && g_y && gamma && save_mean && save_invstd && g_x && g_gamma && g_beta && ws,
                 "dmet_bn_bwd_f32: null pointer");
    DMET_REQUIRE(aligned16(x) && aligned16(g_y) && aligned16(g_x) && aligned16(gamma) && aligned16(save_mean) &&
                     aligned16(save_invstd),
                 "dmet_bn_bwd_f32: pointers must be 16-byte aligned");
    DMET_REQUIRE(ws_bytes >= dmet_bn_workspace_bytes(N, H), "dmet_bn_bwd_f32: workspace too small");
    hipStream_t st = as_stream(stream);
    float *partial = reinterpret_cast<float *>((reinterpret_cast<uintptr_t>(ws) + 255u) & ~(uintptr_t)255u);
    float *mean_g = partial + (size_t)kBnBlocks * 2 * H, *mean_gx = mean_g + H;
    int64_t rpb;
    const int nb = bn_blocks(N, &rpb);
    hipLaunchKernelGGL((bn_reduce_kernel<1>), dim3(nb), dim3(kBnThreads), 0, st, x, g_y, N, H, save_mean, save_invstd,
                       rpb, partial);
    DMET_LAUNCH_CHECK("bn_reduce_kernel<1>");
    hipLaunchKernelGGL(bn_bwd_finalize_kernel, dim3(1), dim3(1024), 0, st, partial, nb, N, H, g_gamma, g_beta, mean_g,
// ... 65 lines not shown
```

### deepmetv2_amd/dense.py

```python
from __future__ import annotations

from typing import Optional

import os

import torch

from . import _native


class _Linear(torch.autograd.Function):
    @staticmethod
    def forward(ctx, x, weight, bias):
        ctx.save_for_backward(x, weight)
        ctx.has_bias = bias is not None
        return torch.addmm(bias, x, weight.t()) if bias is not None else x @ weight.t()

    @staticmethod
    def backward(ctx, g):
        _native.no_double_backward("_Linear")
        x, weight = ctx.saved_tensors
        g = g.contiguous()
        gx = g @ weight if ctx.needs_input_grad[0] else None
        gw = _native.xty(g, x) if ctx.needs_input_grad[1] else None
        gb = g.sum(0) if (ctx.has_bias and ctx.needs_input_grad[2]) else None
        return gx, gw, gb


class _Embedding(torch.autograd.Function):
    @staticmethod
    def forward(ctx, index, weight):
        ctx.save_for_backward(index)
        ctx.rows = weight.shape[0]
        return weight.index_select(0, index)

    @staticmethod
    def backward(ctx, g):
        _native.no_double_backward("_Embedding")
        (index,) = ctx.saved_tensors
        return None, _native.onehot_xty(index, g.contiguous(), ctx.rows)


def linear(x: torch.Tensor, weight: torch.Tensor, bias: Optional[torch.Tensor] = None) -> torch.Tensor:
    if x.dim() != 2 or weight.shape[0] > 64 or weight.shape[1] > 64 or x.dtype != torch.float32:
        return torch.nn.functional.linear(x, weight, bias)
    return _Linear.apply(x, weight, bias)


def embedding(index: torch.Tensor, weight: torch.Tensor) -> torch.Tensor:
    if weight.shape[0] > 64 or weight.shape[1] > 64 or index.dim() != 1:
        return torch.nn.functional.embedding(index, weight)
    return _Embedding.apply(index, weight)


class _Encode(torch.autograd.Function):

    @staticmethod
    def forward(ctx, x_cont, x_cat, *params):
        h = _native.encode_fwd(x_cont, x_cat, [p.detach() for p in params])
        ctx.save_for_backward(x_cont, x_cat, h, *params)
        return h

    @staticmethod
    def backward(ctx, g_h):
        _native.no_double_backward("_Encode")
        x_cont, x_cat, h, *params = ctx.saved_tensors
        grads = _native.encode_bwd(x_cont, x_cat, [p.detach() for p in params], h, g_h.contiguous())
        return (None, None, *grads)


def encode(x_cont: torch.Tensor, x_cat: torch.Tensor, *params: torch.Tensor) -> torch.Tensor:
    return _Encode.apply(x_cont, x_cat, *params)


def _bn_forward(x, residual, gamma, beta, running_mean, running_var, training, momentum, eps, tracked, next_build):
    if next_build is None:
        return _native.bn_fwd(x, residual, gamma, beta, eps, momentum, running_mean, running_var, training,
                              num_batches_tracked=tracked)
    if training:
        mean, invstd = _native.bn_stats(x, eps, momentum, running_mean, running_var, tracked)
    else:
        mean, invstd = _native.bn_eval_stats(running_mean, running_var, eps)
    y = next_build(x, residual, gamma, beta, mean, invstd)
    if y is None:
        y = _native.bn_apply(x, residual, gamma, beta, mean, invstd)
    return y, mean, invstd


class _BatchNorm(torch.autograd.Function):

    @staticmethod
    def forward(ctx, x, residual, weight, bias, running_mean, running_var, training, momentum, eps, tracked=None,
                next_build=None):
        fused = next_build is not None and x.is_cuda and x.shape[1] == 32 and (training or running_mean is not None)
        y, mean, invstd = _bn_forward(x, residual, weight.detach(), bias.detach(), running_mean, running_var, training,
                                      momentum, eps, tracked, next_build if fused else None)
        ctx.save_for_backward(x, weight, mean, invstd)
        ctx.training = training
        ctx.has_residual = residual is not None
        return y

    @staticmethod
    def backward(ctx, g_y):
        _native.no_double_backward("_BatchNorm")
        x, weight, mean, invstd = ctx.saved_tensors
        g_y = g_y.contiguous()
        if ctx.training:
            g_x, g_w, g_b = _native.bn_bwd(x, g_y, weight.detach(), mean, invstd)
        else:
            scale = weight.detach() * invstd
            g_x = g_y * scale
            g_w = (g_y * (x - mean) * invstd).sum(0)
            g_b = g_y.sum(0)
        return g_x, (g_y if ctx.has_residual else None), g_w, g_b, None, None, None, None, None, None, None


ENC_BN_FUSE = os.environ.get("DMET_ENC_BN_FUSE", "1")


class _EncodeBN(torch.autograd.Function):

    @staticmethod
    def forward(ctx, x_cont, x_cat, weight, bias, running_mean, running_var, momentum, eps, tracked, next_build, *params):
        h = _native.encode_fwd(x_cont, x_cat, [p.detach() for p in params])
        y, mean, invstd = _bn_forward(h, None, weight.detach(), bias.detach(), running_mean, running_var, True, momentum, eps,
                                      tracked, next_build)
        ctx.save_for_backward(x_cont, x_cat, h, weight, mean, invstd, *params)
        return y

    @staticmethod
    def backward(ctx, g_y):
        _native.no_double_backward("_EncodeBN")
        x_cont, x_cat, h, weight, mean, invstd, *params = ctx.saved_tensors
        g_y = g_y.contiguous()
        ps = [p.detach() for p in params]
        res = _native.encode_bn_bwd(x_cont, x_cat, ps, h, g_y, weight.detach(), mean, invstd)
        if res is None:
            g_h, g_w, g_b = _native.bn_bwd(h, g_y, weight.detach(), mean, invstd)
            grads = _native.encode_bwd(x_cont, x_cat, ps, h, g_h)
        else:
            grads, g_w, g_b = res
        return (None, None, g_w, g_b, None, None, None, None, None, None, *grads)


def encode_bn(x_cont: torch.Tensor, x_cat: torch.Tensor, bn: torch.nn.BatchNorm1d, next_build, *params: torch.Tensor):
    ok = (ENC_BN_FUSE != "0" and x_cont.is_cuda and bn.training and bn.affine and bn.momentum is not None
          and bn.track_running_stats and bn.num_features == 32 and x_cont.shape[0] > 1)
    if not ok:
        return batch_norm(encode(x_cont, x_cat, *params), bn, next_build=next_build)
    return _EncodeBN.apply(x_cont, x_cat, bn.weight, bn.bias, bn.running_mean, bn.running_var, float(bn.momentum),
                           float(bn.eps), bn.num_batches_tracked, next_build, *params)


def batch_norm(x: torch.Tensor, bn: torch.nn.BatchNorm1d, residual: Optional[torch.Tensor] = None,
               next_build=None) -> torch.Tensor:
    H = x.shape[1] if x.dim() == 2 else -1
    ok = (x.dim() == 2 and x.dtype == torch.float32 and H % 4 == 0 and 4 <= H <= 64 and bn.affine
          and bn.momentum is not None and x.shape[0] > 1 and (bn.training or bn.track_running_stats))
    if not ok:
        own = getattr(bn, "_torch_forward", None)
        y = own(x) if own is not None else bn(x)
        return y if residual is None else residual + y
    training = bn.training or not bn.track_running_stats
    rm = bn.running_mean if bn.track_running_stats else None
    rv = bn.running_var if bn.track_running_stats else None
    tracked = bn.num_batches_tracked if (bn.training and bn.track_running_stats) else None
    return _BatchNorm.apply(x, residual, bn.weight, bn.bias, rm, rv, training, float(bn.momentum), float(bn.eps), tracked,
                            next_build)


_HEAD_PREBUILT = [None]
HEAD_FUSE = os.environ.get("DMET_BN_HEAD_FUSE", "1")


def head_prebuild_hook(W1: torch.Tensor, b1: torch.Tensor, W2: torch.Tensor, b2: torch.Tensor):
    if HEAD_FUSE == "0":
        return None

    def build(raw, residual, gamma, beta, mean, invstd):
        if not raw.is_cuda or raw.dim() != 2 or raw.shape[1] != 32 or raw.dtype != torch.float32:
            return None
        res = _native.bn_head_fwd(raw, residual, gamma, beta, mean, invstd,
                                  [W1.detach(), b1.detach(), W2.detach(), b2.detach()])
        if res is None:
            return None
        _HEAD_PREBUILT[0] = res
        return res[0]
    return build


class _Head(torch.autograd.Function):

    @staticmethod
    def forward(ctx, emb, W1, b1, W2, b2):
        pre, _HEAD_PREBUILT[0] = _HEAD_PREBUILT[0], None
        if pre is not None and pre[0].data_ptr() == emb.data_ptr() and pre[0].shape == emb.shape:
            out = pre[1]
        else:
            out = _native.head_fwd(emb, [W1.detach(), b1.detach(), W2.detach(), b2.detach()])
# ... 15 lines not shown
```

### deepmetv2_amd/graph.py

```python
from __future__ import annotations

import weakref
from typing import Dict, Optional, Tuple

import torch

from . import _native


class BatchInfo:
    __slots__ = ("ptr", "num_events", "num_nodes", "max_nodes", "min_nodes", "inferred")

    def __init__(self, ptr: torch.Tensor, num_events: int, num_nodes: int, max_nodes: Optional[int] = None,
                 min_nodes: Optional[int] = None, inferred: bool = False):
        self.ptr = ptr
        self.num_events = num_events
        self.num_nodes = num_nodes
        self.max_nodes = max_nodes
        self.min_nodes = min_nodes
        self.inferred = inferred


_batch_registry: Dict[int, Tuple[weakref.ref, int, BatchInfo]] = {}

# ... 178 lines not shown
    src = src64.to(torch.int32).contiguous()
    rowptr, perm = _reverse_of_column(tgt, num_nodes)
    ident = torch.arange(E, dtype=torch.int32, device=dev)
    if num_src is None:
        grouped, lo, hi = torch.stack([(perm[:E] == ident).all().to(torch.int64), edge_index.min(),
                                       edge_index.max()]).tolist()
        if lo < 0 or hi >= num_nodes:
            raise ValueError(f"edge_index node ids must lie in [0, {num_nodes}), found {lo if lo < 0 else hi}")
    else:
        grouped, lo, hi, slo, shi = torch.stack([(perm[:E] == ident).all().to(torch.int64), tgt64.min(), tgt64.max(),
                                                 src64.min(), src64.max()]).tolist()
        if lo < 0 or hi >= num_nodes:
            raise ValueError(f"edge_index target ids must lie in [0, {num_nodes}), found {lo if lo < 0 else hi}")
        if slo < 0 or shi >= num_src:
            raise ValueError(f"edge_index source ids must lie in [0, {num_src}), found {slo if slo < 0 else shi}")
    if grouped:
        return EdgeList(src, tgt, rowptr, num_nodes, None, num_src=num_src)
    p = perm[:E].to(torch.int64)
    return EdgeList(src[p].contiguous(), tgt[p].contiguous(), rowptr, num_nodes, perm[:E], num_src=num_src)


class NeighborTable:

    def __init__(self, nbr: Optional[torch.Tensor], ptr: Optional[torch.Tensor], dense: bool, dist: Optional[torch.Tensor] = None,
                 max_nodes: Optional[int] = None, cnt: Optional[torch.Tensor] = None,
                 nbr_local: Optional[torch.Tensor] = None, nonempty: bool = False,
                 rows16: Optional[torch.Tensor] = None, full_rows: bool = False, shape: Optional[Tuple[int, int]] = None):
        if nbr is None and (shape is None or rows16 is None or cnt is None or ptr is None):
            raise ValueError("NeighborTable without an int32 table needs shape, rows16, cnt and ptr")
        self._nbr = nbr
        self.full_rows = full_rows
        self._pending = None
        self.pq = None
        self.rows16 = rows16
        self.nonempty = nonempty
        self._order = None
        self.nbr_local = nbr_local
        self.ptr = ptr
        self.max_nodes = max_nodes
        self.cnt = cnt
        self.num_nodes, self.k = (nbr.shape if nbr is not None else shape)
        self.dense = dense
        self.dist = dist
        self._rev = None
        self._rp = None
        self._rp_full = None
        self._edges = None
        self._edge_index = {}

    @property
    def nbr(self) -> torch.Tensor:
        if self._nbr is None:
            self.join()
            N, k = self.num_nodes, self.k
            counts = (self.ptr[1:] - self.ptr[:-1])
            lo = torch.repeat_interleave(self.ptr[:-1], counts, output_size=N).to(torch.int32).view(-1, 1)
            loc = self.rows16[:, :k].to(torch.int32) & 0xFFFF
            slot = torch.arange(k, device=loc.device, dtype=torch.int32).view(1, -1)
            self._nbr = torch.where(slot < self.cnt.view(-1, 1), loc + lo, torch.full_like(loc, -1)).contiguous()
        return self._nbr

    def has_int32_table(self) -> bool:
        return self._nbr is not None

    def join(self) -> "NeighborTable":
        if self._pending is not None:
# ... 162 lines not shown
```

### deepmetv2_amd/model.py

```python
from __future__ import annotations

import os
from typing import Optional

import torch
from torch import nn

from . import dense
from .conv import DynamicEdgeConv, EdgeConv
from .scatter import met_loss, met_loss_from_weights, met_reduce

PDG_CLASSES = (1, 2, 11, 13, 22, 130, 211)


def _run(seq: nn.Sequential, x: torch.Tensor) -> torch.Tensor:
    for layer in seq:
        x = dense.linear(x, layer.weight, layer.bias) if isinstance(layer, nn.Linear) else layer(x)
    return x


class GraphMETNetwork(nn.Module):
    def __init__(self, continuous_dim: int, cat_dim: int, output_dim: int = 1, hidden_dim: int = 32,
                 conv_depth: int = 1, graph: str = "static", k: int = 16, edge_dtype=None):
        super().__init__()
        if graph not in ("static", "dynamic"):
            raise ValueError("graph must be 'static' or 'dynamic'")
        q, h = hidden_dim // 4, hidden_dim // 2
        self.graph, self.k = graph, k
        self.fused_encoder = os.environ.get("DMET_FUSED_ENCODER", "1") != "0"
        self.embed_charge = nn.Embedding(3, q)
        self.embed_pdgid = nn.Embedding(len(PDG_CLASSES), q)
        self.embed_pv = nn.Embedding(8, q)
        self.embed_continuous = nn.Sequential(nn.Linear(continuous_dim, h), nn.ELU())
        self.embed_categorical = nn.Sequential(nn.Linear(3 * q, h), nn.ELU())
        self.encode_all = nn.Sequential(nn.Linear(hidden_dim, hidden_dim), nn.ELU())
        self.bn_all = nn.BatchNorm1d(hidden_dim)
        self.conv_continuous = nn.ModuleList()
        for _ in range(conv_depth):
            message = nn.Sequential(nn.Linear(2 * hidden_dim, hidden_dim))
            conv = DynamicEdgeConv(nn=message, k=k) if graph == "dynamic" else EdgeConv(nn=message).jittable()
            conv.compute_dtype = edge_dtype
            self.conv_continuous.append(nn.ModuleList([conv, nn.BatchNorm1d(hidden_dim)]))
        self.output = nn.Sequential(nn.Linear(hidden_dim, h), nn.ELU(), nn.Linear(h, output_dim))
        self.pdgs = list(PDG_CLASSES)

    def _fused_encoder_ok(self, x_cont: torch.Tensor, x_cat: torch.Tensor) -> bool:
        return (self.fused_encoder and x_cont.dtype == torch.float32 and x_cont.shape[1] == 8
                and x_cat.shape[1] == 3 and self.encode_all[0].weight.shape == (32, 32)
                and list(self.pdgs) == list(PDG_CLASSES) and not x_cont.requires_grad)

    def _next_build(self, layer: int, batch, graph=None):
        if layer >= len(self.conv_continuous):
            return None
        hook = getattr(self.conv_continuous[layer][0], "prebuild_hook", None)
        if hook is None:
            return None
        return hook(batch) if self.graph == "dynamic" else hook(batch, graph=graph)

    def embed(self, x_cont: torch.Tensor, x_cat: torch.Tensor, batch=None, fuse_next: bool = False, graph=None) -> torch.Tensor:
        if self._fused_encoder_ok(x_cont, x_cat):
            lc, lk, la = self.embed_continuous[0], self.embed_categorical[0], self.encode_all[0]
            return dense.encode_bn(x_cont, x_cat, self.bn_all, self._next_build(0, batch, graph) if fuse_next else None,
                                   lc.weight, lc.bias, lk.weight, lk.bias, la.weight, la.bias,
                                   self.embed_charge.weight, self.embed_pdgid.weight, self.embed_pv.weight)
        if x_cat.is_floating_point():
            x_cat = x_cat.long()
        e_cont = _run(self.embed_continuous, x_cont)
        e_chrg = dense.embedding(x_cat[:, 1] + 1, self.embed_charge.weight)
        e_pv = dense.embedding(x_cat[:, 2], self.embed_pv.weight)
        pdg = x_cat[:, 0].abs()
        for cls, val in enumerate(self.pdgs):
            pdg = torch.where(pdg == val, torch.full_like(pdg, cls), pdg)
        e_pdg = dense.embedding(pdg, self.embed_pdgid.weight)
        e_cat = _run(self.embed_categorical, torch.cat([e_chrg, e_pdg, e_pv], dim=1))
        return dense.batch_norm(_run(self.encode_all, torch.cat([e_cat, e_cont], dim=1)), self.bn_all)

    def _fused_head_ok(self, emb: torch.Tensor) -> bool:
        l1, l2 = self.output[0], self.output[2]
        return (self.fused_encoder and emb.dtype == torch.float32 and emb.shape[1] == 32 and l1.bias is not None
                and l2.bias is not None and tuple(l1.weight.shape) == (16, 32) and tuple(l2.weight.shape) == (1, 16))

    def forward(self, x_cont, x_cat, edge_index, batch, apply_sigmoid: bool = False):
        emb = self.embed(x_cont, x_cat, batch, fuse_next=True, graph=edge_index)
        for layer, (conv, norm) in enumerate(self.conv_continuous):
            msg, res = conv.forward_with_residual_input(emb, batch if self.graph == "dynamic" else edge_index)
            nb = self._next_build(layer + 1, batch, edge_index)
            if nb is None and layer + 1 == len(self.conv_continuous) and apply_sigmoid and self._fused_head_ok(res):
                l1, l2 = self.output[0], self.output[2]
                nb = dense.head_prebuild_hook(l1.weight, l1.bias, l2.weight, l2.bias)
            emb = dense.batch_norm(msg, norm, residual=res, next_build=nb)
        if apply_sigmoid and self._fused_head_ok(emb):
            l1, l2 = self.output[0], self.output[2]
            return dense.head(emb, l1.weight, l1.bias, l2.weight, l2.bias)
        out = _run(self.output, emb).squeeze(-1)
        return torch.sigmoid(out) if apply_sigmoid else out


class Net(nn.Module):

    def __init__(self, continuous_dim: int, categorical_dim: int, graph: str = "static", k: int = 16, edge_dtype=None):
        super().__init__()
        self.graphnet = GraphMETNetwork(continuous_dim, categorical_dim, output_dim=1, hidden_dim=32,
                                        conv_depth=2, graph=graph, k=k, edge_dtype=edge_dtype)

    def forward(self, x_cont, x_cat, edge_index, batch):
        return self.graphnet(x_cont, x_cat, edge_index, batch, apply_sigmoid=True)


def loss_fn(weights: torch.Tensor, prediction: torch.Tensor, truth: torch.Tensor, batch: torch.Tensor,
            ptr: Optional[torch.Tensor] = None) -> torch.Tensor:
    if weights.dtype in (torch.float16, torch.bfloat16):
        weights = weights.float()
    if weights.dtype == torch.float32 and prediction.dtype == torch.float32 and truth.dtype == torch.float32:
        return met_loss_from_weights(weights, prediction, truth, batch, ptr=ptr)
    met = met_reduce(weights, prediction, batch, ptr=ptr, num_events=truth.shape[0])
    return met_loss(met, truth)


def split_features(x: torch.Tensor, lazy_cat: bool = False):
    return x[:, :8], (x[:, 8:] if lazy_cat else x[:, 8:].long())
```

### include/dmet.h

```cpp
#ifndef DMET_H_
#define DMET_H_

#include <stddef.h>
#include <stdint.h>

#ifdef __cplusplus
extern "C" {
#endif

typedef void *dmet_stream_t;

#define DMET_VERSION 1
#define DMET_MAX_K 64
#define DMET_MAX_KNN_DIM 64
#define DMET_MAX_H 128

int dmet_version(void);
const char *dmet_last_error(void);
int dmet_device_available(void);

size_t dmet_knn_workspace_bytes(int64_t N, int B, int D, int k);
int dmet_knn_f32(const float *x, const int64_t *ptr, int B, int64_t N, int D, int k, int32_t *nbr,
                 float *dist, void *ws, size_t ws_bytes, dmet_stream_t stream);
int dmet_knn_local_f32(const float *x, const int64_t *ptr, int B, int64_t N, int D, int k, int32_t *nbr,
// ... 33 lines not shown
int dmet_radius_periodic_f32(const float *x, const int64_t *ptr, int B, int64_t N, int D, float r, int max_nbr,
                             int skip_self, int fill, const float *period, int32_t *nbr, int32_t *cnt,
                             dmet_stream_t stream);
int dmet_radius_windowed_periodic_f32(const float *x, const int64_t *ptr, int B, int64_t N, int D, float r, int max_nbr,
                                      int skip_self, int fill, const float *period, int32_t *nbr, int32_t *cnt,
                                      uint16_t *nbr16, int stride16, void *ws, size_t ws_bytes, dmet_stream_t stream);
int dmet_radius_xy_f32(const float *x, const int64_t *ptr_x, int64_t Nx, const float *y, const int64_t *ptr_y, int64_t Ny,
                       int B, int D, float r, int max_nbr, const float *period, int fill, int32_t *nbr, int32_t *cnt,
                       dmet_stream_t stream);

size_t dmet_edgeconv_linear_workspace_bytes(int64_t N, int Hout);
int dmet_edgeconv_linear_max_fwd_f32(const float *x, const int32_t *nbr, const int64_t *ptr, int B,
                                     int64_t N, int k, int Hin, int Hout, const float *W,
                                     const float *b, float *out, uint8_t *arg, void *ws,
                                     size_t ws_bytes, dmet_stream_t stream);
int dmet_edgeconv_fused_lds_f32(const float *x, const int32_t *nbr, const int64_t *ptr, int B, int64_t N, int k,
                                int Hin, int Hout, const float *W, const float *b, float *out, uint8_t *arg,
                                dmet_stream_t stream);
int dmet_node_linear_split_f32(const float *x, int64_t N, int Hin, int Hout, const float *W,
                               const float *b, float *P, float *Q, dmet_stream_t stream);
int dmet_gather_max_f32(const float *P, const float *Q, const int32_t *nbr, const int64_t *ptr, int B,
                        int64_t N, int k, int H, float *out, uint8_t *arg, dmet_stream_t stream);
int dmet_node_linear_split_sliced_f32(const float *x, int64_t N, int Hin, int Hout, const float *W,
                                      const float *b, float *P, float *Q, dmet_stream_t stream);
int dmet_bn_node_linear_split_f32(const float *raw, const float *residual, const float *gamma, const float *beta,
                                  const float *mean, const float *invstd, float *y, int64_t N, int H, const float *W,
                                  const float *b, int sliced, float *P, float *Q, dmet_stream_t stream);
int dmet_gather_max_lds_sliced_f32(const float *P, const float *Q, const int32_t *nbr, const uint16_t *nbr_local,
                                   const int64_t *ptr, int B, int64_t N, int k, int H, float *out, uint8_t *arg,
                                   dmet_stream_t stream);
int dmet_gather_max_lds_sliced_cap_f32(const float *P, const float *Q, const int32_t *nbr, const uint16_t *nbr_local,
                                       const int64_t *ptr, int B, int64_t N, int k, int H, float *out, uint8_t *arg,
                                       int64_t max_nodes, dmet_stream_t stream);
int dmet_gather_max_counted_f32(const float *P, const float *Q, const int32_t *nbr, const int32_t *cnt, int64_t N,
                                int k, int H, float *out, uint8_t *arg, dmet_stream_t stream);
int dmet_gather_max_lds_f32(const float *P, const float *Q, const int32_t *nbr, const int64_t *ptr, int B,
                            int64_t N, int k, int H, float *out, uint8_t *arg, dmet_stream_t stream);
int dmet_gather_max_counted_lds_f32(const float *P, const float *Q, const int32_t *nbr, const int32_t *cnt,
                                    const int64_t *ptr, int B, int64_t N, int k, int H, int pq_sliced, float *out,
                                    uint8_t *arg, dmet_stream_t stream);
int dmet_table_order_by_count(const int32_t *cnt, const int64_t *ptr, int B, int64_t N, int32_t *order,
                              dmet_stream_t stream);
int dmet_gather_max_counted_lds_j16_f32(const float *P, const float *Q, const int32_t *nbr, const int32_t *cnt,
                                        const int32_t *order, const int64_t *ptr, int B, int64_t N, int k, int H,
                                        int pq_sliced, float *out, uint16_t *argj, dmet_stream_t stream);
int dmet_gather_max_local_j16_f32(const float *P, const float *Q, const uint16_t *nbr16, int stride16,
                                  const int32_t *cnt, const int32_t *order, const int64_t *ptr, int B, int64_t N,
                                  int kmax, int H, int pq_sliced, float *out, uint16_t *argj, dmet_stream_t stream);
int dmet_gather_max_bwd_j16_f32(const float *g_out, const uint16_t *argj, const int64_t *ptr, int B, int64_t N, int H,
                                float *gQ, dmet_stream_t stream);
int dmet_gather_max_lds16_f32(const float *P, const float *Q, const int32_t *nbr, const uint16_t *nbr_local,
                              const int64_t *ptr, int B, int64_t N, int k, int H, float *out, uint8_t *arg,
                              dmet_stream_t stream);
int dmet_gather_max_mixed_f32(const float *P, const float *Q, const int32_t *nbr, const uint16_t *nbr_local,
                              const int64_t *ptr, int B, int64_t N, int k, int H, float *out, uint8_t *arg,
                              dmet_stream_t stream);
int dmet_edge_mlp2_supported(int Hin, int H1, int H2, int k);
int dmet_edge_mlp2_bf16(const float *x, int64_t N, int Hin, const int32_t *nbr, int k, const float *W1, const float *b1,
                        int H1, const float *W2, const float *b2, int H2, int act2, int aggr, float *out,
                        dmet_stream_t stream);
size_t dmet_edge_mlp2_bn_workspace_bytes(int64_t N, int H2);
int dmet_edge_mlp2_bn_bf16(const float *x, int64_t N, int Hin, const int32_t *nbr, int k, const float *W1, const float *b1,
                           int H1, const float *W2, const float *b2, int H2, int act2, int aggr, const float *gamma,
                           const float *beta, float eps, float momentum, float *running_mean, float *running_var,
                           int64_t *num_batches_tracked, int training, float *out, void *ws, size_t ws_bytes,
                           dmet_stream_t stream);
// ... 166 lines not shown
                                  float *g_x_dst, dmet_stream_t stream);

int dmet_met_reduce_f32(const float *w, const float *x, int64_t x_stride, const int64_t *ptr, int B,
                        float *met, dmet_stream_t stream);
int dmet_met_reduce_bwd_f32(const float *g_met, const float *x, int64_t x_stride, const int64_t *ptr,
                            int B, int64_t N, float *g_w, dmet_stream_t stream);
int dmet_adamw_f32(float *param, const float *grad, float *exp_avg, float *exp_avg_sq, float *step, double *bias_pow,
                   int64_t n, double lr, double beta1, double beta2, double eps, double weight_decay,
                   dmet_stream_t stream);
int dmet_adamw_lr_f32(float *param, const float *grad, float *exp_avg, float *exp_avg_sq, float *step, double *bias_pow,
                      int64_t n, const double *lr_dev, double beta1, double beta2, double eps, double weight_decay,
                      dmet_stream_t stream);
int dmet_met_loss_f32(const float *met, const float *truth, int B, float *loss, float *g_met, dmet_stream_t stream);
int dmet_met_loss_strided_f32(const float *met, const float *truth, int64_t truth_stride, int B, float *loss,
                              float *g_met, dmet_stream_t stream);
int dmet_met_reduce_bwd_scaled_f32(const float *g_met, const float *scale, const float *x, int64_t x_stride,
                                   const int64_t *ptr, int B, int64_t N, float *g_w, dmet_stream_t stream);
int dmet_segment_sum_1d_f32(const float *src, const int64_t *ptr, int B, float *out,
                            dmet_stream_t stream);
int dmet_table_degree(const int32_t *nbr, const int32_t *cnt, int64_t N, int k, int32_t *deg, dmet_stream_t stream);
int dmet_table_edges(const int32_t *nbr, const int32_t *cnt, const int32_t *rowptr, int64_t N, int k, int swap,
                     int64_t *first, int64_t *second, int32_t *src32, int32_t *tgt32, dmet_stream_t stream);
int dmet_batch_to_ptr(const int64_t *batch, int64_t N, int B, int64_t *ptr, dmet_stream_t stream);

size_t dmet_xty_workspace_bytes(int64_t N, int Ha, int Hb);
int dmet_xty_f32(const float *A, const float *B, int64_t N, int Ha, int Hb, float *C, void *ws,
                 size_t ws_bytes, dmet_stream_t stream);
int dmet_onehot_xty_f32(const int64_t *index, const float *B, int64_t N, int R, int Hb, float *C, void *ws,
                        size_t ws_bytes, dmet_stream_t stream);

int dmet_encode_fwd_f32(const float *x, int64_t x_stride, const int64_t *x_cat, int64_t N, const float *Wc, const float *bc,
                        const float *Wk, const float *bk, const float *Wa, const float *ba, const float *Echg,
                        const float *Epdg, const float *Epv, float *h, dmet_stream_t stream);
size_t dmet_encode_bwd_workspace_bytes(int64_t N);
int dmet_encode_bwd_f32(const float *x, int64_t x_stride, const int64_t *x_cat, int64_t N, const float *Wc, const float *bc,
                        const float *Wk, const float *bk, const float *Wa, const float *ba, const float *Echg,
                        const float *Epdg, const float *Epv, const float *h, const float *g_h, float *gWc,
                        float *gbc, float *gWk, float *gbk, float *gWa, float *gba, float *gEchg, float *gEpdg,
                        float *gEpv, void *ws, size_t ws_bytes, dmet_stream_t stream);
int dmet_encode_bn_bwd_f32(const float *x, int64_t x_stride, const int64_t *xcat, int64_t N, const float *Wc,
                           const float *bc, const float *Wk, const float *bk, const float *Wa, const float *ba,
                           const float *Echg, const float *Epdg, const float *Epv, const float *h, const float *g_y,
                           const float *bn_gamma, const float *bn_mean, const float *bn_invstd, const float *bn_mean_g,
                           const float *bn_mean_gx, float *gWc, float *gbc, float *gWk, float *gbk, float *gWa,
                           float *gba, float *gEchg, float *gEpdg, float *gEpv, int *fused, void *ws, size_t ws_bytes,
                           dmet_stream_t stream);

size_t dmet_edgeconv_linear_bwd_workspace_bytes(int64_t N, int H);
int dmet_edgeconv_linear_bwd_f32(const float *x, const float *W, const float *g_out, const uint8_t *arg,
                                 const float *gQ, int64_t N, int H, float *gx, float *gW, float *gb, void *ws,
                                 size_t ws_bytes, dmet_stream_t stream);
int dmet_edgeconv_linear_bwd_add_f32(const float *x, const float *W, const float *g_out, const uint8_t *arg,
                                     const float *gQ, const float *g_add, int64_t N, int H, float *gx, float *gW,
                                     float *gb, void *ws, size_t ws_bytes, dmet_stream_t stream);
int dmet_edgeconv_linear_bwd_add_j16_f32(const float *x, const float *W, const float *g_out, const uint16_t *argj,
                                         const float *gQ, const float *g_add, int64_t N, int H, float *gx, float *gW,
                                         float *gb, void *ws, size_t ws_bytes, dmet_stream_t stream);

size_t dmet_bn_workspace_bytes(int64_t N, int H);
int dmet_bn_fwd_f32(const float *x, const float *residual, int64_t N, int H, const float *gamma, const float *beta,
                    float eps, float momentum, float *running_mean, float *running_var, int training, float *y,
                    float *save_mean, float *save_invstd, void *ws, size_t ws_bytes, dmet_stream_t stream);
int dmet_bn_fwd_tracked_f32(const float *x, const float *residual, int64_t N, int H, const float *gamma,
                            const float *beta, float eps, float momentum, float *running_mean, float *running_var,
                            int64_t *num_batches_tracked, int training, float *y, float *save_mean, float *save_invstd,
                            void *ws, size_t ws_bytes, dmet_stream_t stream);
int dmet_bn_bwd_stats_f32(const float *x, const float *g_y, int64_t N, int H, const float *save_mean,
                          const float *save_invstd, float *g_gamma, float *g_beta, float *mean_g, float *mean_gx,
                          void *ws, size_t ws_bytes, dmet_stream_t stream);
int dmet_bn_eval_stats_f32(const float *running_mean, const float *running_var, int H, float eps, float *save_mean,
                           float *save_invstd, dmet_stream_t stream);
int dmet_bn_apply_f32(const float *x, const float *residual, int64_t N, int H, const float *gamma, const float *beta,
                      const float *mean, const float *invstd, float *y, dmet_stream_t stream);
int dmet_bn_stats_f32(const float *x, int64_t N, int H, float eps, float momentum, float *running_mean, float *running_var,
                      int64_t *num_batches_tracked, float *save_mean, float *save_invstd, void *ws, size_t ws_bytes,
                      dmet_stream_t stream);
int dmet_bn_bwd_f32(const float *x, const float *g_y, int64_t N, int H, const float *gamma, const float *save_mean,
                    const float *save_invstd, float *g_x, float *g_gamma, float *g_beta, void *ws, size_t ws_bytes,
                    dmet_stream_t stream);

int dmet_head_fwd_f32(const float *emb, int64_t N, const float *W1, const float *b1, const float *W2, const float *b2,
                      float *out, dmet_stream_t stream);
int dmet_bn_head_fwd_f32(const float *raw, const float *residual, const float *gamma, const float *beta,
                         const float *mean, const float *invstd, float *emb, int64_t N, const float *W1,
                         const float *b1, const float *W2, const float *b2, float *out, int *fused,
                         dmet_stream_t stream);
size_t dmet_head_bwd_workspace_bytes(int64_t N);
int dmet_head_bwd_f32(const float *emb, int64_t N, const float *W1, const float *b1, const float *W2, const float *out,
                      const float *g_out, float *g_emb, float *gW1, float *gb1, float *gW2, float *gb2, void *ws,
                      size_t ws_bytes, dmet_stream_t stream);

int dmet_finalize_defer_begin(void);
int dmet_finalize_pending(void);
int dmet_finalize_flush(dmet_stream_t stream);

#define DMET_GRACLUS_LDS_NODES 16384
#define DMET_GRACLUS_DEFAULT_ROUNDS 64
#define DMET_MAX_CUT_DIM 64
size_t dmet_graclus_workspace_bytes(int64_t N);
int dmet_graclus_f32(const int64_t *rowptr, const int32_t *col, const float *weight, const int64_t *ptr, int B,
                     int64_t N, uint64_t seed, int max_rounds, int64_t *cluster, int32_t *partner, int32_t *rounds,
                     void *ws, size_t ws_bytes, dmet_stream_t stream);
size_t dmet_normalized_cut_workspace_bytes(int64_t N);
int dmet_normalized_cut_f32(const int64_t *row, const int64_t *col, int64_t E, int64_t N, const float *attr, float *w,
                            void *ws, size_t ws_bytes, dmet_stream_t stream);
int dmet_normalized_cut_2d_f32(const int64_t *row, const int64_t *col, int64_t E, int64_t N, const float *x, int D,
                               float *w, void *ws, size_t ws_bytes, dmet_stream_t stream);
size_t dmet_pool_pairs_workspace_bytes(int64_t N, int B);
int dmet_pool_pairs_index(const int32_t *partner, const int64_t *ptr, int B, int64_t N, int64_t *cid,
// ... 39 lines not shown
```

Measured before the change: 53250.

## Fuse BatchNorm moment accumulation into encoder and gather-max kernels

The encoder forward and the LDS gather-max kernel now accumulate per-event, pivot-shifted first and second moments of their outputs. A small finalize kernel combines these into the BatchNorm mean, invstd and running statistics, so the separate full pass over the activations to compute BN stats is skipped in training. This adds reductions and extra LDS syncs inside the producer kernels, plus a Python routing layer that decides when the fused path applies, and it carries some risk to numerical accuracy.

```diff
diff --git a/deepmetv2_amd/_lib.py b/deepmetv2_amd/_lib.py
--- a/deepmetv2_amd/_lib.py
+++ b/deepmetv2_amd/_lib.py
@@ -56,6 +56,7 @@
     "dmet_gather_max_counted_lds_f32": (_i, [_vp, _vp, _vp, _vp, _vp, _i, _i64, _i, _i, _i, _vp, _vp, _vp]),
     "dmet_gather_max_lds_sliced_f32": (_i, [_vp, _vp, _vp, _vp, _vp, _i, _i64, _i, _i, _vp, _vp, _vp]),
     "dmet_gather_max_lds_sliced_cap_f32": (_i, [_vp, _vp, _vp, _vp, _vp, _i, _i64, _i, _i, _vp, _vp, _i64, _vp]),
+    "dmet_bn_moments_gather_max_f32": (_i, [_vp, _vp, _vp, _vp, _vp, _i, _i64, _i, _i, _vp, _vp, _i64, _vp, _vp]),
     "dmet_gather_max_lds16_f32": (_i, [_vp, _vp, _vp, _vp, _vp, _i, _i64, _i, _i, _vp, _vp, _vp]),
     "dmet_edge_mlp2_supported": (_i, [_i, _i, _i, _i]),
     "dmet_edge_mlp2_bf16": (_i, [_vp, _i64, _i, _vp, _i, _vp, _vp, _i, _vp, _vp, _i, _i, _i, _vp, _vp]),
@@ -165,6 +166,9 @@
     "dmet_bn_eval_stats_f32": (_i, [_vp, _vp, _i, _f, _vp, _vp, _vp]),
     "dmet_bn_apply_f32": (_i, [_vp, _vp, _i64, _i, _vp, _vp, _vp, _vp, _vp, _vp]),
     "dmet_bn_stats_f32": (_i, [_vp, _i64, _i, _f, _f, _vp, _vp, _vp, _vp, _vp, _vp, _sz, _vp]),
+    "dmet_bn_fwd_finalize_moments_f32": (_i, [_vp, _i, _i, _f, _f, _vp, _vp, _vp, _vp, _vp, _vp]),
+    "dmet_encode_fwd_moments_parts": (_i, [_i64]),
+    "dmet_encode_fwd_moments_f32": (_i, [_vp, _i64, _vp, _i64] + [_vp] * 9 + [_vp, _vp, _vp]),
     "dmet_bn_bwd_f32": (_i, [_vp, _vp, _i64, _i, _vp, _vp, _vp, _vp, _vp, _vp, _vp, _sz, _vp]),
     "dmet_encode_fwd_f32": (_i, [_vp, _i64, _vp, _i64] + [_vp] * 9 + [_vp, _vp]),
     "dmet_encode_bwd_workspace_bytes": (_sz, [_i64]),
diff --git a/deepmetv2_amd/_native.py b/deepmetv2_amd/_native.py
--- a/deepmetv2_amd/_native.py
+++ b/deepmetv2_amd/_native.py
@@ -468,7 +468,7 @@
 def gather_max(P: torch.Tensor, Q: torch.Tensor, nbr: torch.Tensor, ptr: Optional[torch.Tensor],
                want_arg: bool, cnt: Optional[torch.Tensor] = None, lds: bool = False,
                nbr_local: Optional[torch.Tensor] = None, sliced: bool = False, mixed: bool = False,
-               max_nodes: Optional[int] = None) -> Tuple[torch.Tensor, Optional[torch.Tensor]]:
+               max_nodes: Optional[int] = None, moments: bool = False):
     dev = _require_device(P, Q, nbr)
     N, H = _pq_shape(P, sliced)
     k = nbr.shape[1]
@@ -491,6 +491,14 @@
         entry, args = "dmet_gather_max_lds_sliced_cap_f32", table + (local,) + events + tail + (int(max_nodes or 0),)
         note = ("gather_max_lds_kernel (per-event Q slice resident in LDS; slice-major P/Q, "
                 + ("uint16 event-local ids)" if nbr_local is not None else "int32 ids)"))
+        if moments:
+            if not (want_arg and nbr_local is not None):
+                raise ValueError("gather_max: moments need uint16 ids and want_arg")
+            _check_nbr_local(nbr_local, nbr)
+            mom = torch.empty((events[1], H, 4), dtype=torch.float32, device=dev)
+            _gather_run(dev, 'gather_max', note[:-1] + ", BatchNorm moments)", "dmet_bn_moments_gather_max_f32",
+                        *(args + (mom.data_ptr(),)))
+            return out, arg, mom
     elif cnt is not None and lds and lds_form:
         entry = "dmet_gather_max_counted_lds_f32"
         args = table + (cnt.data_ptr(),) + events + (N, k, H, 1 if sliced else 0) + outs
@@ -511,6 +519,8 @@
     else:
         entry, args = "dmet_gather_max_f32", table + events + tail
         note = "gather_max_mlp_kernel (row gathers from L2; events too large for the LDS image)"
+    if moments:
+        raise ValueError("gather_max: moments come out of the slice-major LDS form alone")
     _gather_run(dev, 'gather_max', note, entry, *args)
     return out, arg
 
@@ -2021,7 +2031,10 @@
     return (x if x.stride(1) == 1 else x.contiguous()), x_cat.contiguous()
 
 
-def encode_fwd(x_cont: torch.Tensor, x_cat: torch.Tensor, params) -> torch.Tensor:
+def encode_fwd(x_cont: torch.Tensor, x_cat: torch.Tensor, params, moments: bool = False):
+    if moments:
+        res = _encode_fwd_moments(x_cont, x_cat, params)
+        return res if res is not None else (encode_fwd(x_cont, x_cat, params), None)
     dev = _require_device(x_cont, x_cat)
     L = _lib.load()
     x, xc = _encode_x(x_cont, x_cat)
@@ -2032,6 +2045,23 @@
         _lib.check(L.dmet_encode_fwd_f32(x.data_ptr(), x.stride(0), _ptr(xc), N, *[t.data_ptr() for t in ps],
                                          h.data_ptr(), _stream(dev)), "dmet_encode_fwd_f32")
     return h
+
+
+def _encode_fwd_moments(x_cont: torch.Tensor, x_cat: torch.Tensor, params):
+    dev = _require_device(x_cont, x_cat)
+    L = _lib.load()
+    x, xc = _encode_x(x_cont, x_cat)
+    ps = _encode_params(params, dev)
+    N = x.shape[0]
+    parts = L.dmet_encode_fwd_moments_parts(N)
+    if parts <= 0 or any(t.data_ptr() % 16 for t in ps[6:]):
+        return None
+    h = torch.empty((N, 32), dtype=torch.float32, device=dev)
+    moments = torch.empty((parts, 32, 4), dtype=torch.float32, device=dev)
+    with _on(dev):
+        _lib.check(L.dmet_encode_fwd_moments_f32(x.data_ptr(), x.stride(0), _ptr(xc), N, *[t.data_ptr() for t in ps],
+                                                 h.data_ptr(), moments.data_ptr(), _stream(dev)), "dmet_encode_fwd_moments_f32")
+    return h, moments
 
 
 def encode_bwd(x_cont: torch.Tensor, x_cat: torch.Tensor, params, h: torch.Tensor, g_h: torch.Tensor):
@@ -2132,7 +2162,10 @@
 
 
 def bn_stats(x: torch.Tensor, eps: float, momentum: float, running_mean: Optional[torch.Tensor],
-             running_var: Optional[torch.Tensor], num_batches_tracked: Optional[torch.Tensor] = None):
+             running_var: Optional[torch.Tensor], num_batches_tracked: Optional[torch.Tensor] = None,
+             moments: Optional[torch.Tensor] = None):
+    if moments is not None:
+        return _bn_stats_moments(moments, eps, momentum, running_mean, running_var, num_batches_tracked)
     dev = _require_device(x)
     L = _lib.load()
     x = _f32a(x, "x")
@@ -2144,6 +2177,25 @@
                                        _ptr(running_var), _ptr(num_batches_tracked),
                                        stats[0].data_ptr(), stats[1].data_ptr(), ws.data_ptr(), ws.numel(), _stream(dev)),
                    "dmet_bn_stats_f32")
+    return stats[0], stats[1]
+
+
+BN_MOMENTS = os.environ.get("DMET_BN_MOMENTS", "1")
+
+
+def _bn_stats_moments(moments: torch.Tensor, eps: float, momentum: float, running_mean: Optional[torch.Tensor],
+                      running_var: Optional[torch.Tensor], num_batches_tracked: Optional[torch.Tensor] = None):
+    dev = _require_device(moments)
+    L = _lib.load()
+    if moments.dim() != 3 or moments.shape[2] != 4 or moments.dtype != torch.float32 or not moments.is_contiguous():
+        raise ValueError("bn_stats: moments must be a contiguous float32 [P, H, 4]")
+    P, H = moments.shape[0], moments.shape[1]
+    stats = torch.empty((2, H), dtype=torch.float32, device=dev)
+    with _on(dev):
+        _lib.check(L.dmet_bn_fwd_finalize_moments_f32(moments.data_ptr(), P, H, float(eps), float(momentum),
+                                                      _ptr(running_mean), _ptr(running_var), _ptr(num_batches_tracked),
+                                                      stats[0].data_ptr(), stats[1].data_ptr(), _stream(dev)),
+                   "dmet_bn_fwd_finalize_moments_f32")
     return stats[0], stats[1]
 
 
diff --git a/deepmetv2_amd/conv.py b/deepmetv2_amd/conv.py
--- a/deepmetv2_amd/conv.py
+++ b/deepmetv2_amd/conv.py
@@ -111,8 +111,14 @@
                 P, Q = pq[0], pq[1]
             else:
                 P, Q = _native.node_linear_split(x, weight, bias, sliced=sliced)
-            out, arg = _native.gather_max(P, Q, table.nbr, table.ptr, want_arg=need_grad, lds=lds,
-                                          nbr_local=table.nbr_local, sliced=sliced, mixed=mixed, max_nodes=table.max_nodes)
+            table.moments = None
+            if table.want_moments and sliced and need_grad and table.nbr_local is not None and not mixed:
+                out, arg, table.moments = _native.gather_max(P, Q, table.nbr, table.ptr, want_arg=True, lds=lds,
+                                                             nbr_local=table.nbr_local, sliced=True,
+                                                             max_nodes=table.max_nodes, moments=True)
+            else:
+                out, arg = _native.gather_max(P, Q, table.nbr, table.ptr, want_arg=need_grad, lds=lds,
+                                              nbr_local=table.nbr_local, sliced=sliced, mixed=mixed, max_nodes=table.max_nodes)
         if need_grad:
             ctx.save_for_backward(x, weight, arg)
             ctx.table = table
@@ -642,13 +648,24 @@
             table = knn_table(x, self.k, batch, loop=True, dense=self._dense_request(x))
         return self._forward_table(x, table)
 
-    def forward_with_residual_input(self, x: torch.Tensor, batch: Optional[torch.Tensor] = None):
+    def forward_with_residual_input(self, x: torch.Tensor, batch: Optional[torch.Tensor] = None, want_moments: bool = False):
+        self._moments = None
         if x.dim() != 2 or x.dtype != torch.float32:
             return self.forward(x, batch), x
         table = self._take_prebuilt(x)
         if table is None:
             table = knn_table(x, self.k, batch, loop=True, dense=self._dense_request(x))
-        return self._forward_table(x, table, passthrough=True)
+        table.want_moments = bool(want_moments)
+        res = self._forward_table(x, table, passthrough=True)
+        if table.moments is not None:
+            self._moments, table.moments = (res[0], table.moments), None
+        return res
+
+    def take_moments(self, out: torch.Tensor) -> Optional[torch.Tensor]:
+        pre, self._moments = getattr(self, "_moments", None), None
+        if pre is not None and pre[0] is out:
+            return pre[1]
+        return None
 
     def prebuild_hook(self, batch: Optional[torch.Tensor] = None, graph=None):
         if BN_KNN_FUSE == "0" or self.k > 20 or os.environ.get("DMET_KNN_PATH") == "exact":
diff --git a/deepmetv2_amd/csrc/common.h b/deepmetv2_amd/csrc/common.h
--- a/deepmetv2_amd/csrc/common.h
+++ b/deepmetv2_amd/csrc/common.h
@@ -79,6 +79,33 @@
     return v;
 }
 
+template <int NV, int CUR, int D, int LAST>
+__device__ __forceinline__ int halving_step(double (&s)[NV], int lane)
+{
+    if constexpr (D > LAST) {
+        return 0;
+    } else {
+        const bool up = (lane & D) != 0;
+        if constexpr (CUR > 1) {
+            constexpr int HALF = CUR / 2;
+#pragma unroll
+            for (int u = 0; u < HALF; ++u) {
+                const double send = up ? s[u] : s[u + HALF], keep = up ? s[u + HALF] : s[u];
+                s[u] = keep + __shfl_xor(send, D, 64);
+            }
+            return (up ? HALF : 0) + halving_step<NV, HALF, 2 * D, LAST>(s, lane);
+        } else {
+            s[0] += __shfl_xor(s[0], D, 64);
+            return halving_step<NV, 1, 2 * D, LAST>(s, lane);
+        }
+    }
+}
+template <int NV, int FIRST, int LAST>
+__device__ __forceinline__ int halving_reduce(double (&s)[NV], int lane)
+{
+    return halving_step<NV, NV, FIRST, LAST>(s, lane);
+}
+
 template <int... Vs, typename F>
 bool with_int(int v, F &&f)
 {
diff --git a/deepmetv2_amd/csrc/edgeconv.hip b/deepmetv2_amd/csrc/edgeconv.hip
--- a/deepmetv2_amd/csrc/edgeconv.hip
+++ b/deepmetv2_amd/csrc/edgeconv.hip
@@ -299,17 +299,24 @@
     }
 }
 
-template <bool WITH_ARG, int K4, int GML_MODE, bool IDS16, bool SLICED, int ROWS = kLdsGatherRows, int THREADS = kLdsGatherThreads>
+template <bool WITH_ARG, int K4, int GML_MODE, bool IDS16, bool SLICED, int ROWS = kLdsGatherRows, int THREADS = kLdsGatherThreads,
+          bool MOMENTS = false>
 __device__ __forceinline__ void gather_max_lds_segment(
     float4 *__restrict__ qs, const float *__restrict__ P, const float *__restrict__ Q, const int32_t *__restrict__ nbr,
     const uint16_t *__restrict__ nbr16, const int64_t *__restrict__ ptr, int k, int H,
     float *__restrict__ out, uint8_t *__restrict__ arg, int64_t N, int skip_big, const int b, const int sl, const int i0,
-    const int i1)
+    const int i1, float *__restrict__ moments = nullptr)
 {
     static_assert(K4 >= 1 && K4 <= 8, "k = 4 K4 <= 32");
     constexpr int RPI = THREADS / 2;
     const int lo = (int)ptr[b], hi = (int)ptr[b + 1];
     const int n = hi - lo;
+    if (MOMENTS && n <= 0) {
+        if (threadIdx.x < 8)
+            reinterpret_cast<float4 *>(moments)[((int64_t)b * (H / 4) + sl * 2 + (threadIdx.x & 1)) * 4 + (threadIdx.x >> 1)] =
+                make_float4(0.f, 0.f, 0.f, 0.f);
+        return;
+    }
     if (n <= 0 || i0 >= i1) return;
     const int h4 = H / 4;
     const float4 *Q4 = reinterpret_cast<const float4 *>(Q);
@@ -319,9 +326,47 @@
     const int col4 = sl * 2 + half;
     const float ninf = -__builtin_inff();
     auto pq_at = [&](const int64_t i) -> int64_t { return SLICED ? ((int64_t)sl * N + i) * 2 + half : i * h4 + col4; };
+    float4 piv = make_float4(0.f, 0.f, 0.f, 0.f), m1 = piv, m2 = piv;
+    auto set_pivot = [&](const float4 a, const float4 c) {
+        const float big = __builtin_inff();
+        piv = make_float4(a.x + c.x, a.y + c.y, a.z + c.z, a.w + c.w);
+        if (!(__builtin_fabsf(piv.x) < big)) piv.x = 0.f;
+        if (!(__builtin_fabsf(piv.y) < big)) piv.y = 0.f;
+        if (!(__builtin_fabsf(piv.z) < big)) piv.z = 0.f;
+        if (!(__builtin_fabsf(piv.w) < big)) piv.w = 0.f;
+    };
+    auto vote = [&](const float4 o) {
+        const float dx = o.x - piv.x, dy = o.y - piv.y, dz = o.z - piv.z, dw = o.w - piv.w;
+        m1.x += dx; m1.y += dy; m1.z += dz; m1.w += dw;
+        m2.x = __builtin_fmaf(dx, dx, m2.x); m2.y = __builtin_fmaf(dy, dy, m2.y);
+        m2.z = __builtin_fmaf(dz, dz, m2.z); m2.w = __builtin_fmaf(dw, dw, m2.w);
+    };
+    auto write_moments = [&]() {
+        double s[8] = {m1.x, m1.y, m1.z, m1.w, m2.x, m2.y, m2.z, m2.w};
+        const int lane = threadIdx.x & 63, wave = threadIdx.x >> 6;
+        const int u_mine = halving_reduce<8, 2, 32>(s, lane);
+        __syncthreads();
+        double *red = reinterpret_cast<double *>(qs);
+        if (lane < 16) red[(wave * 2 + half) * 8 + u_mine] = s[0];
+        __syncthreads();
+        if (threadIdx.x < 64) {
+            const int u = (threadIdx.x >> 1) & 7, ch = u & 3;
+            double sum = 0.0;
+            for (int w = 0; w < THREADS / 64; ++w) sum += red[(w * 2 + half) * 8 + u];
+            const double s1 = sum, s2 = __shfl_down(sum, 8);
+            if (threadIdx.x >= 8) return;
+            const float pf = ch == 0 ? piv.x : ch == 1 ? piv.y : ch == 2 ? piv.z : piv.w;
+            const double pc = (double)pf;
+            const float centre = pf + (float)s1 / (float)n;
+            const double dl = (double)centre - pc;
+            reinterpret_cast<float4 *>(moments)[((int64_t)b * h4 + col4) * 4 + ch] =
+                make_float4((float)n, centre, (float)(s1 - (double)n * dl), (float)(s2 - 2.0 * dl * s1 + (double)n * dl * dl));
+        }
+    };
 
     if (n + 1 > ROWS) {
         if (skip_big) return;
+        if constexpr (MOMENTS) set_pivot(P4[pq_at(lo)], Q4[pq_at(lo)]);
         for (int r = r0; r < i1; r += RPI) {
             const int64_t node = lo + r;
             float4 best = make_float4(ninf, ninf, ninf, ninf);
@@ -343,10 +388,12 @@
                 o = make_float4(p.x + best.x, p.y + best.y, p.z + best.z, p.w + best.w);
             }
             reinterpret_cast<float4 *>(out)[node * h4 + col4] = o;
+            if constexpr (MOMENTS) vote(o);
             if (WITH_ARG)
                 reinterpret_cast<uchar4 *>(arg)[node * h4 + col4] =
                     make_uchar4((unsigned char)a0, (unsigned char)a1, (unsigned char)a2, (unsigned char)a3);
         }
+        if constexpr (MOMENTS) write_moments();
         return;
     }
 
@@ -378,6 +425,7 @@
     __syncthreads();
     if (threadIdx.x < 2) qs[n * 2 + threadIdx.x] = make_float4(ninf, ninf, ninf, ninf);
     __syncthreads();
+    if constexpr (MOMENTS) set_pivot(P4[pq_at(lo)], qs[half]);
 
     for (int r = r0; r < i1; r += RPI) {
         const int64_t node = lo + r;
@@ -486,11 +534,13 @@
         float4 o = make_float4(0.f, 0.f, 0.f, 0.f);
         if (any) o = make_float4(p.x + bx, p.y + by, p.z + bz, p.w + bw);
         reinterpret_cast<float4 *>(out)[node * h4 + col4] = o;
+        if constexpr (MOMENTS) vote(o);
         if (WITH_ARG) {
             const uchar4 a = make_uchar4((unsigned char)a0, (unsigned char)a1, (unsigned char)a2, (unsigned char)a3);
             reinterpret_cast<uchar4 *>(arg)[node * h4 + col4] = a;
         }
     }
+    if constexpr (MOMENTS) write_moments();
 }
 
 inline int num_cus()
@@ -508,11 +558,11 @@
 }
 
 template <bool WITH_ARG, int K4, int GML_MODE = 0, bool IDS16 = false, bool SLICED = false, int ROWS = kLdsGatherRows,
-          int THREADS = kLdsGatherThreads>
+          int THREADS = kLdsGatherThreads, bool MOMENTS = false>
 __global__ __launch_bounds__(THREADS) void gather_max_lds_kernel(
     const float *__restrict__ P, const float *__restrict__ Q, const int32_t *__restrict__ nbr,
     const uint16_t *__restrict__ nbr16, const int64_t *__restrict__ ptr, int B, int k, int H,
-    float *__restrict__ out, uint8_t *__restrict__ arg, int64_t N, int skip_big, int balanced)
+    float *__restrict__ out, uint8_t *__restrict__ arg, int64_t N, int skip_big, int balanced, float *__restrict__ moments)
 {
     __shared__ __attribute__((aligned(16))) float4 qs[ROWS * 2];
     const int nsl = H / kSliceC;
@@ -521,10 +571,11 @@
         const int b = grp * kNumXcd + (rem % kNumXcd);
         const int sl = rem / kNumXcd;
         if (b >= B) return;
-        gather_max_lds_segment<WITH_ARG, K4, GML_MODE, IDS16, SLICED, ROWS, THREADS>(qs, P, Q, nbr, nbr16, ptr, k, H, out, arg, N,
-                                                                                      skip_big, b, sl, 0, (int)(ptr[b + 1] - ptr[b]));
+        gather_max_lds_segment<WITH_ARG, K4, GML_MODE, IDS16, SLICED, ROWS, THREADS, MOMENTS>(
+            qs, P, Q, nbr, nbr16, ptr, k, H, out, arg, N, skip_big, b, sl, 0, (int)(ptr[b + 1] - ptr[b]), moments);
         return;
     }
+    if constexpr (MOMENTS) return;
     const int64_t L = (int64_t)nsl * N;
     const int c = xcd_swizzle((int)blockIdx.x, (int)gridDim.x);
     int64_t pos = L * c / gridDim.x;
@@ -1144,6 +1195,7 @@
     bool pq_sliced = false;
     int skip_big = 0;
     int64_t max_nodes = 0;
+    float *moments = nullptr;
 };
 
 int gather_max_launch(const GatherMax &r)
@@ -1166,6 +1218,9 @@
     DMET_REQUIRE(aligned16(r.P) && aligned16(r.Q) && aligned16(r.out) && (fam != kGatherLds || aligned16(r.nbr)) &&
                      (fam == kGatherL2 || aligned16(r.nbr16)) && (!r.arg16 || (reinterpret_cast<uintptr_t>(r.arg) & 7u) == 0),
                  "%s: pointers must be 16-B (uint16 winners: 8-B) aligned", r.entry);
+    DMET_REQUIRE(!r.moments || (fam == kGatherLds && k_lds && r.pq_sliced && r.nbr16 && r.arg && !r.arg16 && !r.skip_big),
+                 "%s: moments need the slice-major LDS form with uint16 ids and winners, k in {8,16,20,32}", r.entry);
+    DMET_REQUIRE(aligned16(r.moments), "%s: moments must be 16-B aligned", r.entry);
     hipStream_t st = as_stream(r.stream);
     uint8_t *arg = static_cast<uint8_t *>(r.arg);
     const int nsl = H / kSliceC;
@@ -1200,7 +1255,7 @@
         const int64_t units = (int64_t)B * nsl;
         int balanced = units * 16 <= (int64_t)cus * 9 || (units > cus && units % cus != 0 && units % cus <= cus / 8);
         if (const char *e = getenv("DMET_GATHER_BALANCED")) balanced = atoi(e) != 0;
-        if (half) balanced = 0;
+        if (half || r.moments) balanced = 0;
         int64_t blocks = per_event;
         if (balanced) {
             blocks = cus;
@@ -1213,20 +1268,20 @@
         timed = with_int<1, 2>(e ? atoi(e) : 0, [&](auto mode) {
             hipLaunchKernelGGL((gather_max_lds_kernel<true, 4, decltype(mode)::value, true>), dim3((unsigned)blocks),
                                dim3(kLdsGatherThreads), 0, st, r.P, r.Q, r.nbr, r.nbr16, r.ptr, B, k, H, r.out, arg, N, r.skip_big,
-                               balanced);
+                               balanced, (float *)nullptr);
         });
 #endif
         if (!timed)
             with_int<8, 16, 20, 32>(k, [&](auto kk) {
                 constexpr int K4 = decltype(kk)::value / 4;
-                with_flags([&](auto with_arg, auto ids16, auto sliced, auto small) {
+                with_flags([&](auto with_arg, auto ids16, auto sliced, auto small, auto mom) {
                     constexpr int ROWS = small() ? kLdsGatherRowsHalf : kLdsGatherRows;
                     constexpr int THREADS = small() ? kLdsGatherThreadsHalf : kLdsGatherThreads;
-                    if constexpr (!small() || (ids16() && sliced()))
-                        hipLaunchKernelGGL((gather_max_lds_kernel<with_arg(), K4, 0, ids16(), sliced(), ROWS, THREADS>),
+                    if constexpr ((!small() || (ids16() && sliced())) && (!mom() || (with_arg() && ids16() && sliced())))
+                        hipLaunchKernelGGL((gather_max_lds_kernel<with_arg(), K4, 0, ids16(), sliced(), ROWS, THREADS, mom()>),
                                            dim3((unsigned)blocks), dim3(THREADS), 0, st, r.P, r.Q, r.nbr, r.nbr16, r.ptr, B, k, H, r.out,
-                                           arg, N, r.skip_big, balanced);
-                }, arg != nullptr, r.nbr16 != nullptr, r.pq_sliced, half);
+                                           arg, N, r.skip_big, balanced, r.moments);
+                }, arg != nullptr, r.nbr16 != nullptr, r.pq_sliced, half, r.moments != nullptr);
             });
         DMET_LAUNCH_CHECK(half ? "gather_max_lds_kernel (80 KB image)" : "gather_max_lds_kernel");
         if (!r.skip_big) return 0;
@@ -1311,6 +1366,18 @@
 {
     GatherMax r{"dmet_gather_max_lds_sliced_cap_f32", kGatherLds, P, Q, N, k, H, out, stream};
     r.nbr = nbr; r.nbr16 = nbr_local; r.ptr = ptr; r.B = B; r.arg = arg; r.pq_sliced = true; r.max_nodes = max_nodes;
+    return gather_max_launch(r);
+}
+
+extern "C" int dmet_bn_moments_gather_max_f32(const float *P, const float *Q, const int32_t *nbr,
+                                                          const uint16_t *nbr_local, const int64_t *ptr, int B, int64_t N,
+                                                          int k, int H, float *out, uint8_t *arg, int64_t max_nodes,
+                                                          float *moments, dmet_stream_t stream)
+{
+    DMET_REQUIRE(moments, "dmet_bn_moments_gather_max_f32: null pointer");
+    GatherMax r{"dmet_bn_moments_gather_max_f32", kGatherLds, P, Q, N, k, H, out, stream};
+    r.nbr = nbr; r.nbr16 = nbr_local; r.ptr = ptr; r.B = B; r.arg = arg; r.pq_sliced = true; r.max_nodes = max_nodes;
+    r.moments = moments;
     return gather_max_launch(r);
 }
 
diff --git a/deepmetv2_amd/csrc/encoder.hip b/deepmetv2_amd/csrc/encoder.hip
--- a/deepmetv2_amd/csrc/encoder.hip
+++ b/deepmetv2_amd/csrc/encoder.hip
@@ -83,9 +83,10 @@
         o[c] = make_float4(elu(z3[4 * c]), elu(z3[4 * c + 1]), elu(z3[4 * c + 2]), elu(z3[4 * c + 3]));
 }
 
-__global__ __launch_bounds__(256) void encode_fwd_mfma_kernel(const float *__restrict__ x, int64_t x_stride,
-                                                               const int64_t *__restrict__ xcat, int64_t N, ENC_PARAMS,
-                                                               float *__restrict__ h)
+template <bool MOMENTS>
+__device__ __forceinline__ void encode_fwd_mfma_body(const float *__restrict__ x, int64_t x_stride,
+                                                     const int64_t *__restrict__ xcat, int64_t N, ENC_PARAMS,
+                                                     float *__restrict__ h, float *__restrict__ moments)
 {
     const int lane = threadIdx.x & 63, r = lane & 31, hh = lane >> 5;
     const int64_t wave = (int64_t)blockIdx.x * (blockDim.x >> 6) + __builtin_amdgcn_readfirstlane((int)(threadIdx.x >> 6));
@@ -130,6 +131,12 @@
     };
     Raw raw;
     float in[16], nxt[16];
+    float piv[16], m1[16], m2[16];
+    int votes = 0;
+    if constexpr (MOMENTS) {
+#pragma unroll
+        for (int e = 0; e < 16; ++e) { piv[e] = 0.0f; m1[e] = 0.0f; m2[e] = 0.0f; }
+    }
     if (wave < ntiles) { load_raw(wave, raw); load_tables(raw, in); }
     if (wave + nwaves < ntiles) load_raw(wave + nwaves, raw);
     for (int64_t tile = wave; tile < ntiles; tile += nwaves) {
@@ -148,15 +155,90 @@
         for (int e = 0; e < 16; ++e) acc[e] = b3[e];
 #pragma unroll
         for (int s = 0; s < 16; ++s) acc = __builtin_amdgcn_mfma_f32_32x32x2f32(w3[s], joint[s], acc, 0, 0, 0);
-        if (node < N) {
-            float4 *o = reinterpret_cast<float4 *>(h + node * 32 + 4 * hh);
-#pragma unroll
-            for (int g = 0; g < 4; ++g)
-                o[2 * g] = make_float4(elu(acc[4 * g]), elu(acc[4 * g + 1]), elu(acc[4 * g + 2]), elu(acc[4 * g + 3]));
+        if constexpr (!MOMENTS) {
+            if (node < N) {
+                float4 *o = reinterpret_cast<float4 *>(h + node * 32 + 4 * hh);
+#pragma unroll
+                for (int g = 0; g < 4; ++g)
+                    o[2 * g] = make_float4(elu(acc[4 * g]), elu(acc[4 * g + 1]), elu(acc[4 * g + 2]), elu(acc[4 * g + 3]));
+            }
+        } else {
+            float v[16];
+#pragma unroll
+            for (int e = 0; e < 16; ++e) v[e] = elu(acc[e]);
+            if (tile == wave) {
+#pragma unroll
+                for (int e = 0; e < 16; ++e) {
+                    const float p = __shfl(v[e], hh * 32);
+                    piv[e] = __builtin_fabsf(p) < __builtin_inff() ? p : 0.0f;
+                }
+            }
+            if (node < N) {
+                float4 *o = reinterpret_cast<float4 *>(h + node * 32 + 4 * hh);
+#pragma unroll
+                for (int g = 0; g < 4; ++g) o[2 * g] = make_float4(v[4 * g], v[4 * g + 1], v[4 * g + 2], v[4 * g + 3]);
+                ++votes;
+#pragma unroll
+                for (int e = 0; e < 16; ++e) {
+                    const float d = v[e] - piv[e];
+                    m1[e] += d;
+                    m2[e] = __builtin_fmaf(d, d, m2[e]);
+                }
+            }
         }
 #pragma unroll
         for (int u = 0; u < 16; ++u) in[u] = nxt[u];
     }
+    if constexpr (MOMENTS) {
+        __shared__ double red[4][2][49];
+        const int wv = threadIdx.x >> 6;
+#pragma unroll
+        for (int d = 1; d < 32; d <<= 1) votes += __shfl_xor(votes, d);
+        double s[32];
+#pragma unroll
+        for (int e = 0; e < 16; ++e) { s[e] = (double)m1[e]; s[16 + e] = (double)m2[e]; }
+        const int mine = halving_reduce<32, 1, 16>(s, lane);
+        red[wv][hh][17 + mine] = s[0];
+        if (r == 0) {
+            red[wv][hh][0] = (double)votes;
+#pragma unroll
+            for (int e = 0; e < 16; ++e) red[wv][hh][1 + e] = (double)piv[e];
+        }
+        __syncthreads();
+        if (threadIdx.x < 32) {
+            const int e = threadIdx.x & 15, half = threadIdx.x >> 4;
+            const int ch = (e & 3) + 8 * (e >> 2) + 4 * half;
+            const double p0 = red[0][half][1 + e];
+            double n = 0.0, s1 = 0.0, s2 = 0.0;
+            for (int w = 0; w < 4; ++w) {
+                const double *q = red[w][half];
+                const double nw = q[0], dl = q[1 + e] - p0, a = q[17 + e], c = q[33 + e];
+                if (nw > 0.0) {
+                    n += nw;
+                    s1 += a + nw * dl;
+                    s2 += c + 2.0 * dl * a + nw * dl * dl;
+                }
+            }
+            const float centre = (float)(p0 + s1 / n);
+            const double dc = (double)centre - p0;
+            reinterpret_cast<float4 *>(moments)[(int64_t)blockIdx.x * 32 + ch] =
+                make_float4((float)n, centre, (float)(s1 - n * dc), (float)(s2 - 2.0 * dc * s1 + n * dc * dc));
+        }
+    }
+}
+
+__global__ __launch_bounds__(256) void encode_fwd_mfma_kernel(const float *__restrict__ x, int64_t x_stride,
+                                                               const int64_t *__restrict__ xcat, int64_t N, ENC_PARAMS,
+                                                               float *__restrict__ h)
+{
+    encode_fwd_mfma_body<false>(x, x_stride, xcat, N, ENC_ARGS, h, nullptr);
+}
+
+__global__ __launch_bounds__(256) void encode_fwd_mfma_moments_kernel(const float *__restrict__ x, int64_t x_stride,
+                                                                       const int64_t *__restrict__ xcat, int64_t N, ENC_PARAMS,
+                                                                       float *__restrict__ h, float *__restrict__ moments)
+{
+    encode_fwd_mfma_body<true>(x, x_stride, xcat, N, ENC_ARGS, h, moments);
 }
 
 constexpr int kEncTiles = 3;
@@ -612,6 +694,15 @@
     return npw;
 }
 
+inline int64_t enc_fwd_mfma_grid(int64_t N)
+{
+    const int64_t tiles = (N + 31) / 32;
+    int64_t grid = (tiles + 3) / 4;
+    int gmax = 512;
+    if (const char *e = getenv("DMET_ENC_GRID")) { gmax = atoi(e); if (gmax < 1) gmax = 512; }
+    return grid > gmax ? gmax : grid;
+}
+
 thread_local EncBnBwd g_enc_bnb{nullptr, nullptr, nullptr, nullptr, nullptr};
 thread_local bool g_enc_bnb_done = false;
 
@@ -634,11 +725,7 @@
     DMET_REQUIRE(blocks < (1ll << 31), "dmet_encode_fwd_f32: too many nodes");
     const int form = env_is("DMET_ENCODER_FWD", "valu") ? 0 : 1;
     if (form == 1 && aligned16(Echg) && aligned16(Epdg) && aligned16(Epv)) {
-        const int64_t tiles = (N + 31) / 32;
-        int64_t grid = (tiles + 3) / 4;
-        int gmax = 512;
-        if (const char *e = getenv("DMET_ENC_GRID")) { gmax = atoi(e); if (gmax < 1) gmax = 512; }
-        if (grid > gmax) grid = gmax;
+        const int64_t grid = enc_fwd_mfma_grid(N);
         hipLaunchKernelGGL(encode_fwd_mfma_kernel, dim3((unsigned)grid), dim3(256), 0, as_stream(stream), x, x_stride, xcat, N,
                            ENC_ARGS, h);
         DMET_LAUNCH_CHECK("encode_fwd_mfma_kernel");
@@ -646,6 +733,32 @@
     }
     hipLaunchKernelGGL(encode_fwd_kernel, dim3((unsigned)blocks), dim3(256), 0, as_stream(stream), x, x_stride, xcat, N, ENC_ARGS, h);
     DMET_LAUNCH_CHECK("encode_fwd_kernel");
+    return 0;
+}
+
+extern "C" int dmet_encode_fwd_moments_parts(int64_t N)
+{
+    if (N <= 0 || env_is("DMET_ENCODER_FWD", "valu")) return 0;
+    return (int)enc_fwd_mfma_grid(N);
+}
+
+extern "C" int dmet_encode_fwd_moments_f32(const float *x, int64_t x_stride, const int64_t *xcat, int64_t N, const float *Wc,
+                                           const float *bc, const float *Wk, const float *bk, const float *Wa, const float *ba,
+                                           const float *Echg, const float *Epdg, const float *Epv, float *h, float *moments,
+                                           dmet_stream_t stream)
+{
+    DMET_REQUIRE(N > 0 && x_stride >= 8, "dmet_encode_fwd_moments_f32: bad sizes");
+    DMET_REQUIRE(x && Wc && bc && Wk && bk && Wa && ba && Echg && Epdg && Epv && h && moments,
+                 "dmet_encode_fwd_moments_f32: null pointer");
+    DMET_REQUIRE(xcat || x_stride >= 11, "dmet_encode_fwd_moments_f32: x_cat == NULL needs rows of at least 11 columns (x_stride=%lld)",
+                 (long long)x_stride);
+    DMET_REQUIRE(aligned16(h) && aligned16(moments) && aligned16(Echg) && aligned16(Epdg) && aligned16(Epv),
+                 "dmet_encode_fwd_moments_f32: h, moments and the embedding tables must be 16-B aligned");
+    DMET_REQUIRE((N + 255) / 256 < (1ll << 31), "dmet_encode_fwd_moments_f32: too many nodes");
+    DMET_REQUIRE(dmet_encode_fwd_moments_parts(N) > 0, "dmet_encode_fwd_moments_f32: the matrix-core forward is switched off");
+    hipLaunchKernelGGL(encode_fwd_mfma_moments_kernel, dim3((unsigned)enc_fwd_mfma_grid(N)), dim3(256), 0, as_stream(stream), x,
+                       x_stride, xcat, N, ENC_ARGS, h, moments);
+    DMET_LAUNCH_CHECK("encode_fwd_mfma_moments_kernel");
     return 0;
 }
 
diff --git a/deepmetv2_amd/csrc/norm.hip b/deepmetv2_amd/csrc/norm.hip
--- a/deepmetv2_amd/csrc/norm.hip
+++ b/deepmetv2_amd/csrc/norm.hip
@@ -100,6 +100,53 @@
     }
 }
 
+__global__ __launch_bounds__(1024) void bn_fwd_finalize_moments_kernel(const float *__restrict__ moments, int P, int H,
+                                                                       float eps, float momentum,
+                                                                       float *__restrict__ running_mean,
+                                                                       float *__restrict__ running_var,
+                                                                       float *__restrict__ save_mean,
+                                                                       float *__restrict__ save_invstd,
+                                                                       int64_t *__restrict__ num_batches_tracked)
+{
+    __shared__ double g0[1024], g1[1024], g2[1024];
+    const int G = 1024 / H;
+    const int c = threadIdx.x % H, grp = threadIdx.x / H;
+    const float4 *m4 = reinterpret_cast<const float4 *>(moments);
+    float4 first = m4[c];
+    double n = 0.0, s1 = 0.0, s2 = 0.0;
+    if (first.x <= 0.f)
+        for (int p = 1; p < P && first.x <= 0.f; ++p) first = m4[(int64_t)p * H + c];
+    const double g = first.x > 0.f ? (double)first.y : 0.0;
+    if (grp < G)
+#pragma unroll 8
+        for (int p = grp; p < P; p += G) {
+            const float4 m = m4[(int64_t)p * H + c];
+            if (m.x > 0.f) {
+                const double np = (double)m.x, dl = (double)m.y - g, a = (double)m.z;
+                n += np;
+                s1 += __builtin_fma(np, dl, a);
+                s2 += __builtin_fma(dl, __builtin_fma(np, dl, a + a), (double)m.w);
+            }
+        }
+    if (grp < G) { g0[grp * H + c] = n; g1[grp * H + c] = s1; g2[grp * H + c] = s2; }
+    __syncthreads();
+    if (threadIdx.x == 0 && num_batches_tracked) *num_batches_tracked += 1;
+    if (threadIdx.x >= H) return;
+    n = 0.0; s1 = 0.0; s2 = 0.0;
+    for (int q = 0; q < G; ++q) { n += g0[q * H + c]; s1 += g1[q * H + c]; s2 += g2[q * H + c]; }
+    const double m = n > 0.0 ? s1 / n : 0.0;
+    double var = n > 0.0 ? s2 / n - m * m : 0.0;
+    if (var < 0.0) var = 0.0;
+    const double mean = g + m;
+    save_mean[c] = (float)mean;
+    save_invstd[c] = (float)(1.0 / sqrt(var + (double)eps));
+    if (running_mean) {
+        const double unbiased = n > 1.0 ? var * n / (n - 1.0) : var;
+        running_mean[c] = (float)((1.0 - (double)momentum) * (double)running_mean[c] + (double)momentum * mean);
+        running_var[c] = (float)((1.0 - (double)momentum) * (double)running_var[c] + (double)momentum * unbiased);
+    }
+}
+
 __global__ __launch_bounds__(64) void bn_eval_stats_kernel(const float *__restrict__ running_mean,
                                                            const float *__restrict__ running_var, int H, float eps,
                                                            float *__restrict__ save_mean,
@@ -238,6 +285,22 @@
     hipLaunchKernelGGL(bn_fwd_finalize_kernel, dim3(1), dim3(1024), 0, st, partial, nb, x, N, H, eps, momentum, running_mean,
                        running_var, save_mean, save_invstd, num_batches_tracked);
     DMET_LAUNCH_CHECK("bn_fwd_finalize_kernel");
+    return 0;
+}
+
+extern "C" int dmet_bn_fwd_finalize_moments_f32(const float *moments, int P, int H, float eps, float momentum,
+                                                float *running_mean, float *running_var, int64_t *num_batches_tracked,
+                                                float *save_mean, float *save_invstd, dmet_stream_t stream)
+{
+    DMET_REQUIRE(bn_shape_ok(H), "dmet_bn_fwd_finalize_moments_f32: H=%d must be a multiple of 4 in [4,64]", H);
+    DMET_REQUIRE(P > 0, "dmet_bn_fwd_finalize_moments_f32: P=%d", P);
+    DMET_REQUIRE(moments && save_mean && save_invstd, "dmet_bn_fwd_finalize_moments_f32: null pointer");
+    DMET_REQUIRE(aligned16(moments), "dmet_bn_fwd_finalize_moments_f32: moments must be 16-byte aligned");
+    DMET_REQUIRE((running_mean == nullptr) == (running_var == nullptr),
+                 "dmet_bn_fwd_finalize_moments_f32: running_mean/var go together");
+    hipLaunchKernelGGL(bn_fwd_finalize_moments_kernel, dim3(1), dim3(1024), 0, as_stream(stream), moments, P, H, eps, momentum,
+                       running_mean, running_var, save_mean, save_invstd, num_batches_tracked);
+    DMET_LAUNCH_CHECK("bn_fwd_finalize_moments_kernel");
     return 0;
 }
 
diff --git a/deepmetv2_amd/dense.py b/deepmetv2_amd/dense.py
--- a/deepmetv2_amd/dense.py
+++ b/deepmetv2_amd/dense.py
@@ -53,11 +53,30 @@
     return _Embedding.apply(index, weight)
 
 
+_ASK_MOMENTS = [False]
+_MOMENTS = [None]
+
+
+def _encode_forward(x_cont, x_cat, ps):
+    ask, _ASK_MOMENTS[0] = _ASK_MOMENTS[0], False
+    if ask:
+        return _native.encode_fwd(x_cont, x_cat, ps, moments=True)
+    return _native.encode_fwd(x_cont, x_cat, ps), None
+
+
+def _take_moments(x):
+    pre, _MOMENTS[0] = _MOMENTS[0], None
+    if pre is not None and pre[0].data_ptr() == x.data_ptr() and pre[0].shape == x.shape:
+        return pre[1]
+    return None
+
+
 class _Encode(torch.autograd.Function):
 
     @staticmethod
     def forward(ctx, x_cont, x_cat, *params):
-        h = _native.encode_fwd(x_cont, x_cat, [p.detach() for p in params])
+        h, moments = _encode_forward(x_cont, x_cat, [p.detach() for p in params])
+        _MOMENTS[0] = (h, moments) if moments is not None else None
         ctx.save_for_backward(x_cont, x_cat, h, *params)
         return h
 
@@ -73,7 +92,14 @@
     return _Encode.apply(x_cont, x_cat, *params)
 
 
-def _bn_forward(x, residual, gamma, beta, running_mean, running_var, training, momentum, eps, tracked, next_build):
+def _bn_forward(x, residual, gamma, beta, running_mean, running_var, training, momentum, eps, tracked, next_build,
+                moments=None):
+    if moments is not None and training:
+        mean, invstd = _native.bn_stats(x, eps, momentum, running_mean, running_var, tracked, moments=moments)
+        y = next_build(x, residual, gamma, beta, mean, invstd) if next_build is not None else None
+        if y is None:
+            y = _native.bn_apply(x, residual, gamma, beta, mean, invstd)
+        return y, mean, invstd
     if next_build is None:
         return _native.bn_fwd(x, residual, gamma, beta, eps, momentum, running_mean, running_var, training,
                               num_batches_tracked=tracked)
@@ -94,7 +120,7 @@
                 next_build=None):
         fused = next_build is not None and x.is_cuda and x.shape[1] == 32 and (training or running_mean is not None)
         y, mean, invstd = _bn_forward(x, residual, weight.detach(), bias.detach(), running_mean, running_var, training,
-                                      momentum, eps, tracked, next_build if fused else None)
+                                      momentum, eps, tracked, next_build if fused else None, _take_moments(x))
         ctx.save_for_backward(x, weight, mean, invstd)
         ctx.training = training
         ctx.has_residual = residual is not None
@@ -122,9 +148,10 @@
 
     @staticmethod
     def forward(ctx, x_cont, x_cat, weight, bias, running_mean, running_var, momentum, eps, tracked, next_build, *params):
-        h = _native.encode_fwd(x_cont, x_cat, [p.detach() for p in params])
+        _MOMENTS[0] = None
+        h, moments = _encode_forward(x_cont, x_cat, [p.detach() for p in params])
         y, mean, invstd = _bn_forward(h, None, weight.detach(), bias.detach(), running_mean, running_var, True, momentum, eps,
-                                      tracked, next_build)
+                                      tracked, next_build, moments)
         ctx.save_for_backward(x_cont, x_cat, h, weight, mean, invstd, *params)
         return y
 
@@ -143,17 +170,22 @@
         return (None, None, g_w, g_b, None, None, None, None, None, None, *grads)
 
 
-def encode_bn(x_cont: torch.Tensor, x_cat: torch.Tensor, bn: torch.nn.BatchNorm1d, next_build, *params: torch.Tensor):
+def encode_bn(x_cont: torch.Tensor, x_cat: torch.Tensor, bn: torch.nn.BatchNorm1d, next_build, *params: torch.Tensor,
+              want_moments: bool = False):
     ok = (ENC_BN_FUSE != "0" and x_cont.is_cuda and bn.training and bn.affine and bn.momentum is not None
           and bn.track_running_stats and bn.num_features == 32 and x_cont.shape[0] > 1)
+    _ASK_MOMENTS[0] = bool(want_moments and bn.training and x_cont.is_cuda and x_cont.shape[0] > 1)
     if not ok:
-        return batch_norm(encode(x_cont, x_cat, *params), bn, next_build=next_build)
+        h = encode(x_cont, x_cat, *params)
+        _ASK_MOMENTS[0] = False
+        return batch_norm(h, bn, next_build=next_build, moments=_take_moments(h))
     return _EncodeBN.apply(x_cont, x_cat, bn.weight, bn.bias, bn.running_mean, bn.running_var, float(bn.momentum),
                            float(bn.eps), bn.num_batches_tracked, next_build, *params)
 
 
 def batch_norm(x: torch.Tensor, bn: torch.nn.BatchNorm1d, residual: Optional[torch.Tensor] = None,
-               next_build=None) -> torch.Tensor:
+               next_build=None, moments: Optional[torch.Tensor] = None) -> torch.Tensor:
+    _MOMENTS[0] = None
     H = x.shape[1] if x.dim() == 2 else -1
     ok = (x.dim() == 2 and x.dtype == torch.float32 and H % 4 == 0 and 4 <= H <= 64 and bn.affine
           and bn.momentum is not None and x.shape[0] > 1 and (bn.training or bn.track_running_stats))
@@ -165,6 +197,8 @@
     rm = bn.running_mean if bn.track_running_stats else None
     rv = bn.running_var if bn.track_running_stats else None
     tracked = bn.num_batches_tracked if (bn.training and bn.track_running_stats) else None
+    if moments is not None and bn.training:
+        _MOMENTS[0] = (x, moments)
     return _BatchNorm.apply(x, residual, bn.weight, bn.bias, rm, rv, training, float(bn.momentum), float(bn.eps), tracked,
                             next_build)
 
diff --git a/deepmetv2_amd/graph.py b/deepmetv2_amd/graph.py
--- a/deepmetv2_amd/graph.py
+++ b/deepmetv2_amd/graph.py
@@ -234,6 +234,8 @@
         self.full_rows = full_rows
         self._pending = None
         self.pq = None
+        self.want_moments = False
+        self.moments = None
         self.rows16 = rows16
         self.nonempty = nonempty
         self._order = None
diff --git a/deepmetv2_amd/model.py b/deepmetv2_amd/model.py
--- a/deepmetv2_amd/model.py
+++ b/deepmetv2_amd/model.py
@@ -6,8 +6,9 @@
 import torch
 from torch import nn
 
-from . import dense
-from .conv import DynamicEdgeConv, EdgeConv
+from . import _native, dense
+from .conv import _LDS_MAX_EVENT_NODES, DynamicEdgeConv, EdgeConv
+from .graph import batch_info
 from .scatter import met_loss, met_loss_from_weights, met_reduce
 
 PDG_CLASSES = (1, 2, 11, 13, 22, 130, 211)
@@ -57,12 +58,29 @@
             return None
         return hook(batch) if self.graph == "dynamic" else hook(batch, graph=graph)
 
-    def embed(self, x_cont: torch.Tensor, x_cat: torch.Tensor, batch=None, fuse_next: bool = False, graph=None) -> torch.Tensor:
+    def _moments_route(self, x_cont: torch.Tensor, x_cat: torch.Tensor, batch) -> bool:
+        if (_native.BN_MOMENTS == "0" or self.graph != "dynamic" or not self.training or not torch.is_grad_enabled()
+                or not x_cont.is_cuda or batch is None or x_cont.shape[0] < 2 or not self._fused_encoder_ok(x_cont, x_cat)):
+            return False
+        blocks = list(self.conv_continuous)
+        if len(blocks) != 2 or blocks[0] is blocks[1] or blocks[0][0] is blocks[1][0] or blocks[0][1] is blocks[1][1]:
+            return False
+        for bn in [self.bn_all] + [b[1] for b in blocks]:
+            if not (bn.training and bn.affine and bn.track_running_stats and bn.momentum is not None):
+                return False
+        if not all(p.requires_grad for p in self.parameters()):
+            return False
+        info = batch_info(batch, x_cont.shape[0], x_cont.device)
+        return info.max_nodes is not None and info.max_nodes <= _LDS_MAX_EVENT_NODES
+
+    def embed(self, x_cont: torch.Tensor, x_cat: torch.Tensor, batch=None, fuse_next: bool = False, graph=None,
+              want_moments: bool = False) -> torch.Tensor:
         if self._fused_encoder_ok(x_cont, x_cat):
             lc, lk, la = self.embed_continuous[0], self.embed_categorical[0], self.encode_all[0]
             return dense.encode_bn(x_cont, x_cat, self.bn_all, self._next_build(0, batch, graph) if fuse_next else None,
                                    lc.weight, lc.bias, lk.weight, lk.bias, la.weight, la.bias,
-                                   self.embed_charge.weight, self.embed_pdgid.weight, self.embed_pv.weight)
+                                   self.embed_charge.weight, self.embed_pdgid.weight, self.embed_pv.weight,
+                                   want_moments=want_moments)
         if x_cat.is_floating_point():
             x_cat = x_cat.long()
         e_cont = _run(self.embed_continuous, x_cont)
@@ -81,14 +99,19 @@
                 and l2.bias is not None and tuple(l1.weight.shape) == (16, 32) and tuple(l2.weight.shape) == (1, 16))
 
     def forward(self, x_cont, x_cat, edge_index, batch, apply_sigmoid: bool = False):
+        moments = self._moments_route(x_cont, x_cat, batch)
         emb = self.embed(x_cont, x_cat, batch, fuse_next=True, graph=edge_index)
         for layer, (conv, norm) in enumerate(self.conv_continuous):
-            msg, res = conv.forward_with_residual_input(emb, batch if self.graph == "dynamic" else edge_index)
+            if moments:
+                msg, res = conv.forward_with_residual_input(emb, batch, want_moments=True)
+            else:
+                msg, res = conv.forward_with_residual_input(emb, batch if self.graph == "dynamic" else edge_index)
             nb = self._next_build(layer + 1, batch, edge_index)
             if nb is None and layer + 1 == len(self.conv_continuous) and apply_sigmoid and self._fused_head_ok(res):
                 l1, l2 = self.output[0], self.output[2]
                 nb = dense.head_prebuild_hook(l1.weight, l1.bias, l2.weight, l2.bias)
-            emb = dense.batch_norm(msg, norm, residual=res, next_build=nb)
+            emb = dense.batch_norm(msg, norm, residual=res, next_build=nb,
+                                   moments=conv.take_moments(msg) if moments else None)
         if apply_sigmoid and self._fused_head_ok(emb):
             l1, l2 = self.output[0], self.output[2]
             return dense.head(emb, l1.weight, l1.bias, l2.weight, l2.bias)
diff --git a/include/dmet.h b/include/dmet.h
--- a/include/dmet.h
+++ b/include/dmet.h
@@ -89,6 +89,9 @@
 int dmet_gather_max_lds_sliced_cap_f32(const float *P, const float *Q, const int32_t *nbr, const uint16_t *nbr_local,
                                        const int64_t *ptr, int B, int64_t N, int k, int H, float *out, uint8_t *arg,
                                        int64_t max_nodes, dmet_stream_t stream);
+int dmet_bn_moments_gather_max_f32(const float *P, const float *Q, const int32_t *nbr, const uint16_t *nbr_local,
+                                   const int64_t *ptr, int B, int64_t N, int k, int H, float *out, uint8_t *arg,
+                                   int64_t max_nodes, float *moments, dmet_stream_t stream);
 int dmet_gather_max_counted_f32(const float *P, const float *Q, const int32_t *nbr, const int32_t *cnt, int64_t N,
                                 int k, int H, float *out, uint8_t *arg, dmet_stream_t stream);
 int dmet_gather_max_lds_f32(const float *P, const float *Q, const int32_t *nbr, const int64_t *ptr, int B,
@@ -321,6 +324,11 @@
 int dmet_encode_fwd_f32(const float *x, int64_t x_stride, const int64_t *x_cat, int64_t N, const float *Wc, const float *bc,
                         const float *Wk, const float *bk, const float *Wa, const float *ba, const float *Echg,
                         const float *Epdg, const float *Epv, float *h, dmet_stream_t stream);
+int dmet_encode_fwd_moments_parts(int64_t N);
+int dmet_encode_fwd_moments_f32(const float *x, int64_t x_stride, const int64_t *x_cat, int64_t N, const float *Wc,
+                                const float *bc, const float *Wk, const float *bk, const float *Wa, const float *ba,
+                                const float *Echg, const float *Epdg, const float *Epv, float *h, float *moments,
+                                dmet_stream_t stream);
 size_t dmet_encode_bwd_workspace_bytes(int64_t N);
 int dmet_encode_bwd_f32(const float *x, int64_t x_stride, const int64_t *x_cat, int64_t N, const float *Wc, const float *bc,
                         const float *Wk, const float *bk, const float *Wa, const float *ba, const float *Echg,
@@ -364,6 +372,9 @@
 int dmet_bn_stats_f32(const float *x, int64_t N, int H, float eps, float momentum, float *running_mean, float *running_var,
                       int64_t *num_batches_tracked, float *save_mean, float *save_invstd, void *ws, size_t ws_bytes,
                       dmet_stream_t stream);
+int dmet_bn_fwd_finalize_moments_f32(const float *moments, int P, int H, float eps, float momentum, float *running_mean,
+                                     float *running_var, int64_t *num_batches_tracked, float *save_mean,
+                                     float *save_invstd, dmet_stream_t stream);
 int dmet_bn_bwd_f32(const float *x, const float *g_y, int64_t N, int H, const float *gamma, const float *save_mean,
                     const float *save_invstd, float *g_x, float *g_gamma, float *g_beta, void *ws, size_t ws_bytes,
                     dmet_stream_t stream);
```

New measurement: 53890, median of 4. 1.01x the previous value.
